# GemsLab/H2GCN

Measured on AMD Instinct MI355X. Metric: aggregated edges/sec (1+2-hop SpMM), higher is better.
Workload: dtype f32

## Files before the change

### h2gcn_amd/_capi.py

```python
from __future__ import annotations

import ctypes as C
import os
from pathlib import Path

ABI_VERSION = 4
MAX_HOPS = 8

OK = 0
ERR_INVALID_ARGUMENT = -1
ERR_HIP = -2
ERR_OUT_OF_MEMORY = -3
ERR_BAD_INDEX = -4
ERR_NO_TRANSPOSE = -5
ERR_INTERNAL = -6
ERR_EXCHANGE_TIMEOUT = -7

METRICS_MAX_SETS = 4
XCHG_BLOB_BYTES = 192
XCHG_COPY_ENGINE = 0
XCHG_COPY_KERNEL = 1

PLAN_BUILD_TRANSPOSE = 0x1
PLAN_SKIP_VALIDATION = 0x2
PLAN_HOST_TRANSPOSE = 0x4
PLAN_KEEP_PERMUTATION = 0x8

EXPORTED_SYMBOLS = (
    "h2gcn_abi_version",
    "h2gcn_last_error",
    "h2gcn_device_count",
    "h2gcn_plan_create",
    "h2gcn_plan_destroy",
    "h2gcn_plan_info",
    "h2gcn_plan_set_values",
    "h2gcn_spmm_hops_f32",
    "h2gcn_spmm_hops_T_f32",
    "h2gcn_plan_schedule",
    "h2gcn_plan_segment_classes",
    "h2gcn_spmm_workspace_bytes",
    "h2gcn_spmm_hops_opts_f32",
    "h2gcn_spmm_hops_T_opts_f32",
    "h2gcn_ring_scratch_bytes",
    "h2gcn_ring_count",
    "h2gcn_ring_fill",
    "h2gcn_ring_count_rows",
    "h2gcn_ring_fill_rows",
    "h2gcn_hop_normalize",
    "h2gcn_hop_normalize_rows",
    "h2gcn_dropout_dense_small_rows",
    "h2gcn_dropout_dense_workspace_bytes",
    "h2gcn_dropout_dense_f32",
    "h2gcn_dropout_dense_backward_f32",
    "h2gcn_masked_metrics_workspace_bytes",
    "h2gcn_masked_metrics_f32",
    "h2gcn_masked_ce_backward_f32",
    "h2gcn_adam_keras_f32",
    "h2gcn_adam_keras_l2_f32",
    "h2gcn_l2_penalty_workspace_bytes",
    "h2gcn_l2_penalty_f32",
    "h2gcn_xchg_create",
    "h2gcn_xchg_export",
    "h2gcn_xchg_connect",
    "h2gcn_xchg_allgather_begin",
    "h2gcn_xchg_allgather_post",
    "h2gcn_xchg_allgather_pull",
    "h2gcn_xchg_allgather_pull_rows",
    "h2gcn_xchg_allgather_end",
    "h2gcn_xchg_reduce_scatter_begin",
    "h2gcn_xchg_reduce_scatter_end",
    "h2gcn_xchg_reset_dependencies",
    "h2gcn_xchg_status",
    "h2gcn_xchg_destroy",
)


class PlanOpts(C.Structure):
    _fields_ = [
        ("struct_size", C.c_uint32),
        ("flags", C.c_uint32),
        ("long_row_threshold", C.c_int32),
        ("rows_per_wave", C.c_int32),
        ("variant", C.c_int32),
        ("slice_cols", C.c_int32),
        ("reserved", C.c_int32 * 2),
    ]


LAUNCH_RELU = 0x1
LAUNCH_ACCUMULATE = 0x2


class LaunchOpts(C.Structure):
    _fields_ = [
        ("struct_size", C.c_uint32),
        ("flags", C.c_uint32),
        ("workspace", C.c_void_p),
        ("workspace_bytes", C.c_size_t),
        ("bias", C.c_void_p),
    ]


class H2GCNError(RuntimeError):

    def __init__(self, status: int, message: str):
        super().__init__(f"libh2gcn_hip: {message} (status {status})")
        self.status = status


def library_path() -> Path:
    override = os.environ.get("H2GCN_HIP_LIBRARY")
    if override:
        return Path(override)
    return Path(__file__).resolve().parent / "csrc" / "libh2gcn_hip.so"


_LIB = None


def lib() -> C.CDLL:
    global _LIB
    if _LIB is not None:
        return _LIB
    path = library_path()
    if not path.exists():
        raise RuntimeError(
            f"{path} not found: build it with `python -c 'import __graft_entry__ as g; g.build()'` "
            "or `make -C h2gcn_amd/csrc`.  h2gcn_amd has no CPU fallback."
        )
    L = C.CDLL(str(path))
    L.h2gcn_abi_version.restype = C.c_int
    L.h2gcn_abi_version.argtypes = []
    L.h2gcn_last_error.restype = C.c_char_p
    L.h2gcn_last_error.argtypes = []
    L.h2gcn_device_count.restype = C.c_int
    L.h2gcn_device_count.argtypes = []
    L.h2gcn_plan_create.restype = C.c_int
    L.h2gcn_plan_create.argtypes = [
        C.c_int, C.c_int64, C.c_int64,
        C.POINTER(C.c_void_p), C.POINTER(C.c_void_p), C.POINTER(C.c_void_p),
        C.POINTER(PlanOpts), C.c_void_p, C.POINTER(C.c_void_p),
    ]
    L.h2gcn_plan_destroy.restype = None
    L.h2gcn_plan_destroy.argtypes = [C.c_void_p]
    L.h2gcn_plan_set_values.restype = C.c_int
    L.h2gcn_plan_set_values.argtypes = [C.c_void_p, C.c_int, C.c_void_p, C.c_void_p]
    L.h2gcn_plan_info.restype = C.c_int
    L.h2gcn_plan_info.argtypes = [
        C.c_void_p, C.c_int, C.POINTER(C.c_int64), C.POINTER(C.c_int64), C.POINTER(C.c_int64),
        C.POINTER(C.c_int64), C.POINTER(C.c_int32),
    ]
    L.h2gcn_spmm_hops_f32.restype = C.c_int
    L.h2gcn_spmm_hops_f32.argtypes = [
        C.c_void_p, C.c_uint32, C.c_void_p, C.c_int64, C.c_int32, C.c_void_p, C.c_int64, C.c_int64, C.c_void_p,
    ]
    L.h2gcn_spmm_hops_T_f32.restype = C.c_int
    L.h2gcn_spmm_hops_T_f32.argtypes = [
        C.c_void_p, C.c_uint32, C.c_void_p, C.c_int64, C.c_int64, C.c_int32, C.c_void_p, C.c_int64, C.c_void_p,
    ]
    L.h2gcn_plan_schedule.restype = C.c_int
    L.h2gcn_plan_schedule.argtypes = [C.c_void_p, C.c_uint32, C.c_int, C.c_int64, C.c_int32] + [C.POINTER(C.c_int32)] * 4
    if hasattr(L, "h2gcn_plan_segment_classes"):
        L.h2gcn_plan_segment_classes.restype = C.c_int
        L.h2gcn_plan_segment_classes.argtypes = [C.c_void_p, C.c_uint32, C.c_int, C.c_int64, C.c_int32] + [C.POINTER(C.c_int64)] * 3
    L.h2gcn_spmm_workspace_bytes.restype = C.c_size_t
    L.h2gcn_spmm_workspace_bytes.argtypes = [C.c_void_p, C.c_uint32, C.c_int, C.c_void_p, C.c_int64, C.c_int64, C.c_int32]
    L.h2gcn_spmm_hops_opts_f32.restype = C.c_int
    L.h2gcn_spmm_hops_opts_f32.argtypes = [
        C.c_void_p, C.c_uint32, C.c_void_p, C.c_int64, C.c_int32, C.c_void_p, C.c_int64, C.c_int64,
        C.POINTER(LaunchOpts), C.c_void_p,
    ]
    L.h2gcn_spmm_hops_T_opts_f32.restype = C.c_int
    L.h2gcn_spmm_hops_T_opts_f32.argtypes = [
        C.c_void_p, C.c_uint32, C.c_void_p, C.c_int64, C.c_int64, C.c_int32, C.c_void_p, C.c_int64,
        C.POINTER(LaunchOpts), C.c_void_p,
    ]
    L.h2gcn_ring_scratch_bytes.restype = C.c_size_t
    L.h2gcn_ring_scratch_bytes.argtypes = [C.c_int64]
    ring_common = [C.c_int64, C.c_void_p, C.c_void_p, C.c_void_p, C.c_void_p,
                   C.c_int, C.POINTER(C.c_void_p), C.POINTER(C.c_void_p), C.c_int,
                   C.c_int, C.POINTER(C.c_void_p), C.POINTER(C.c_void_p), C.c_int]
    L.h2gcn_ring_count.restype = C.c_int
    L.h2gcn_ring_count.argtypes = ring_common + [C.c_void_p, C.POINTER(C.c_int64), C.c_void_p, C.c_size_t, C.c_void_p]
    L.h2gcn_ring_fill.restype = C.c_int
    L.h2gcn_ring_fill.argtypes = ring_common + [C.c_void_p, C.c_void_p, C.c_void_p, C.c_size_t, C.c_void_p]
    ring_rows = [C.c_int64, C.c_int64, C.c_int64] + ring_common[1:]
    L.h2gcn_ring_count_rows.restype = C.c_int
    L.h2gcn_ring_count_rows.argtypes = ring_rows + [C.c_void_p, C.POINTER(C.c_int64), C.c_void_p, C.c_size_t, C.c_void_p]
    L.h2gcn_ring_fill_rows.restype = C.c_int
    L.h2gcn_ring_fill_rows.argtypes = ring_rows + [C.c_void_p, C.c_void_p, C.c_void_p, C.c_size_t, C.c_void_p]
    L.h2gcn_hop_normalize_rows.restype = C.c_int
    L.h2gcn_hop_normalize_rows.argtypes = [C.c_int64, C.c_void_p, C.c_void_p, C.c_int, C.c_void_p, C.c_int64, C.c_void_p, C.c_void_p, C.c_void_p]
    L.h2gcn_hop_normalize.restype = C.c_int
    L.h2gcn_hop_normalize.argtypes = [C.c_int64, C.c_void_p, C.c_void_p, C.c_int, C.c_void_p, C.c_int64, C.c_void_p, C.c_void_p]
    if hasattr(L, "h2gcn_dropout_dense_small_rows"):
        L.h2gcn_dropout_dense_small_rows.restype = C.c_int64
        L.h2gcn_dropout_dense_small_rows.argtypes = [C.c_int64]
    L.h2gcn_dropout_dense_workspace_bytes.restype = C.c_size_t
    L.h2gcn_dropout_dense_workspace_bytes.argtypes = [C.c_int64, C.c_int32, C.c_int32]
    L.h2gcn_dropout_dense_f32.restype = C.c_int
    L.h2gcn_dropout_dense_f32.argtypes = [C.c_void_p, C.c_int64, C.c_int64, C.c_int32, C.c_void_p, C.c_int32, C.c_void_p, C.c_float,
                                          C.c_uint64, C.c_void_p, C.c_void_p, C.c_int64, C.c_void_p, C.c_size_t, C.c_void_p]
    L.h2gcn_dropout_dense_backward_f32.restype = C.c_int
    L.h2gcn_dropout_dense_backward_f32.argtypes = [C.c_void_p, C.c_int64, C.c_int64, C.c_int32, C.c_void_p, C.c_int32, C.c_void_p, C.c_int64,
                                                   C.c_float, C.c_uint64, C.c_void_p, C.c_void_p, C.c_int64, C.c_void_p, C.c_void_p,
                                                   C.c_size_t, C.c_void_p]
    L.h2gcn_masked_metrics_workspace_bytes.restype = C.c_size_t
    L.h2gcn_masked_metrics_workspace_bytes.argtypes = [C.c_int64]
    L.h2gcn_masked_metrics_f32.restype = C.c_int
    L.h2gcn_masked_metrics_f32.argtypes = [C.c_void_p, C.c_int64, C.c_int64, C.c_int32, C.c_int32, C.POINTER(C.c_void_p), C.POINTER(C.c_int64),
                                           C.POINTER(C.c_void_p), C.c_void_p, C.c_void_p, C.c_void_p, C.c_size_t, C.c_void_p]
    L.h2gcn_masked_ce_backward_f32.restype = C.c_int
    L.h2gcn_masked_ce_backward_f32.argtypes = [C.c_void_p, C.c_int64, C.c_int64, C.c_int32, C.c_void_p, C.c_int64, C.c_void_p, C.c_void_p,
                                               C.c_void_p, C.c_int64, C.c_void_p]
    L.h2gcn_adam_keras_f32.restype = C.c_int
    L.h2gcn_adam_keras_f32.argtypes = [C.c_int32, C.POINTER(C.c_void_p), C.POINTER(C.c_void_p), C.POINTER(C.c_void_p), C.POINTER(C.c_void_p),
                                       C.POINTER(C.c_int64), C.c_float, C.c_float, C.c_float, C.c_float, C.c_void_p, C.c_int64, C.c_void_p]
    if hasattr(L, "h2gcn_adam_keras_l2_f32"):
        L.h2gcn_adam_keras_l2_f32.restype = C.c_int
        L.h2gcn_adam_keras_l2_f32.argtypes = [C.c_int32, C.POINTER(C.c_void_p), C.POINTER(C.c_void_p), C.POINTER(C.c_void_p), C.POINTER(C.c_void_p),
                                              C.POINTER(C.c_int64), C.POINTER(C.c_float), C.c_float, C.c_float, C.c_float, C.c_float, C.c_void_p,
                                              C.c_int64, C.c_void_p]
        L.h2gcn_l2_penalty_workspace_bytes.restype = C.c_size_t
        L.h2gcn_l2_penalty_workspace_bytes.argtypes = []
        L.h2gcn_l2_penalty_f32.restype = C.c_int
        L.h2gcn_l2_penalty_f32.argtypes = [C.c_int32, C.POINTER(C.c_void_p), C.POINTER(C.c_int64), C.POINTER(C.c_float), C.c_void_p, C.c_void_p,
                                           C.c_size_t, C.c_void_p]
    L.h2gcn_xchg_create.restype = C.c_int
    L.h2gcn_xchg_create.argtypes = [C.c_int, C.c_int, C.c_int, C.c_size_t, C.c_int, C.c_int, C.POINTER(C.c_void_p)]
    L.h2gcn_xchg_export.restype = C.c_int
    L.h2gcn_xchg_export.argtypes = [C.c_void_p, C.c_void_p]
    L.h2gcn_xchg_connect.restype = C.c_int
    L.h2gcn_xchg_connect.argtypes = [C.c_void_p, C.c_void_p]
    L.h2gcn_xchg_allgather_begin.restype = C.c_int
    L.h2gcn_xchg_allgather_begin.argtypes = [
        C.c_void_p, C.c_int, C.c_void_p, C.c_int64, C.c_int64, C.c_int64, C.c_int32, C.c_void_p, C.c_void_p,
    ]
    L.h2gcn_xchg_allgather_post.restype = C.c_int
    L.h2gcn_xchg_allgather_post.argtypes = L.h2gcn_xchg_allgather_begin.argtypes
    L.h2gcn_xchg_allgather_pull.restype = C.c_int
    L.h2gcn_xchg_allgather_pull.argtypes = [C.c_void_p, C.c_int, C.c_int64, C.c_int32, C.c_void_p]
    if hasattr(L, "h2gcn_xchg_allgather_pull_rows"):
        L.h2gcn_xchg_allgather_pull_rows.restype = C.c_int
        L.h2gcn_xchg_allgather_pull_rows.argtypes = [C.c_void_p, C.c_int, C.c_int64, C.c_int32, C.c_void_p, C.POINTER(C.c_void_p), C.POINTER(C.c_int64)]
    L.h2gcn_xchg_allgather_end.restype = C.c_int
    L.h2gcn_xchg_allgather_end.argtypes = [C.c_void_p, C.c_int, C.c_void_p]
    L.h2gcn_xchg_reduce_scatter_begin.restype = C.c_int
    L.h2gcn_xchg_reduce_scatter_begin.argtypes = [C.c_void_p, C.c_int, C.c_void_p, C.c_int64, C.c_int32, C.c_void_p, C.c_void_p]
    L.h2gcn_xchg_reduce_scatter_end.restype = C.c_int
    L.h2gcn_xchg_reduce_scatter_end.argtypes = [C.c_void_p, C.c_int, C.c_void_p]
    L.h2gcn_xchg_reset_dependencies.restype = C.c_int
    L.h2gcn_xchg_reset_dependencies.argtypes = [C.c_void_p]
    L.h2gcn_xchg_status.restype = C.c_int
    L.h2gcn_xchg_status.argtypes = [C.c_void_p]
    L.h2gcn_xchg_destroy.restype = None
    L.h2gcn_xchg_destroy.argtypes = [C.c_void_p]
    got = L.h2gcn_abi_version()
    if got != ABI_VERSION and not (os.environ.get("H2GCN_HIP_LIBRARY") and got == 3):
        raise RuntimeError(f"{path}: ABI version {got}, this front end expects {ABI_VERSION}")
    _LIB = L
    return L


def has(symbol: str) -> bool:
    return hasattr(lib(), symbol)


def check(status: int) -> None:
    if status < 0:
        msg = lib().h2gcn_last_error()
        raise H2GCNError(status, msg.decode("utf-8", "replace") if msg else "unknown error")
```

### h2gcn_amd/csrc/h2gcn_capi.hip

```cpp
#include <hip/hip_runtime.h>

#include <algorithm>
#include <cstdarg>
#include <cstdlib>
#include <cstdio>
#include <cstring>
#include <deque>
#include <map>
#include <mutex>
#include <memory>
#include <new>
#include <string>
#include <vector>

#include "h2gcn_hip.h"
#include "spmm_kernels.hip.h"

#include "capi_internal.h"

namespace h2gcn {

thread_local std::string g_last_error;

int fail(h2gcn_status st, const char* fmt, ...) {
    char buf[512];
    va_list ap;
    va_start(ap, fmt);
    vsnprintf(buf, sizeof(buf), fmt, ap);
    va_end(ap);
    g_last_error = buf;
    return (int)st;
}

}

namespace {

using h2gcn::fail;
using h2gcn::g_last_error;

struct DeviceBuf {
    void* p = nullptr;
    ~DeviceBuf() {
        if (p) (void)hipFree(p);
    }
    DeviceBuf() = default;
    DeviceBuf(DeviceBuf&& o) noexcept : p(o.p) { o.p = nullptr; }
    DeviceBuf(const DeviceBuf&) = delete;
    DeviceBuf& operator=(const DeviceBuf&) = delete;
};

struct HopOperand {
    const int64_t* rowptr = nullptr;
    const int32_t* colidx = nullptr;
    const float* vals = nullptr;
    int64_t nnz = 0;
    std::vector<int64_t> long_rows;
    std::vector<uint8_t> len8;
    int64_t n_short = 0, nnz_short = 0;
    int64_t nnz_long = 0;
    const uint32_t* perm = nullptr;
};

struct LongList {
    DeviceBuf dev;
    int n = 0;
    LongList() = default;
    LongList(LongList&&) noexcept = default;
};

struct ClassLists {
    DeviceBuf short_dev, med_dev;
    int64_t n_short = 0, nnz_short = 0, n_med = 0;
    bool built = false;
    ClassLists() = default;
    ClassLists(ClassLists&&) noexcept = default;
};

}

struct h2gcn_plan {
    int n_hops = 0;
    int64_t n_rows = 0, n_cols = 0;
    int long_threshold = 256;
    int rows_per_wave = 4;
    int variant = 0;
    int slice_cols = 0;
    bool has_transpose = false;
    int device = 0;
    std::vector<HopOperand> fwd;
    std::vector<HopOperand> adj;
    std::deque<DeviceBuf> owned;
    mutable std::mutex mu;
    mutable std::map<uint64_t, LongList> long_cache;
    mutable std::map<uint64_t, ClassLists> class_cache;
    int short_max = -1;
    double short_min_frac = 0.05;
};

namespace h2gcn {
__global__ void check_colidx_kernel(const int32_t* __restrict__ colidx, int64_t nnz, int64_t n_cols, int* flag) {
    int bad = 0;
    for (int64_t i = (int64_t)blockIdx.x * blockDim.x + threadIdx.x; i < nnz; i += (int64_t)gridDim.x * blockDim.x) {
        const int32_t c = colidx[i];
        bad |= (c < 0) | ((int64_t)c >= n_cols);
    }
    if (bad) atomicOr(flag, 1);
}

void launch_in_tile_short(bool sum, const LaunchParams& p, int slice, bool off32, bool fb4, dim3 grid, hipStream_t stream);
int transpose_csr_device(int64_t n_rows, int64_t n_cols, int64_t nnz, const int64_t* rowptr, const int32_t* colidx,
                         const float* vals, int64_t** t_rowptr_out, int32_t** t_colidx_out, float** t_vals_out,
                         uint32_t** perm_out_keep, hipStream_t stream, std::string* err);
void permute_values(const uint32_t* perm, const float* vals, int64_t nnz, float* t_vals, hipStream_t stream);
}

namespace {

using h2gcn::HopCsr;
using h2gcn::LaunchParams;

int transpose_csr_host(int64_t n_rows, int64_t n_cols, const std::vector<int64_t>& rowptr,
                       const std::vector<int32_t>& colidx, const std::vector<float>& vals,
                       std::vector<int64_t>& t_rowptr, std::vector<int32_t>& t_colidx, std::vector<float>& t_vals) {
    const int64_t nnz = rowptr[n_rows];
    t_rowptr.assign(n_cols + 1, 0);
    t_colidx.resize(nnz);
    t_vals.resize(nnz);
    for (int64_t i = 0; i < nnz; ++i) t_rowptr[colidx[i] + 1]++;
    for (int64_t c = 0; c < n_cols; ++c) t_rowptr[c + 1] += t_rowptr[c];
    std::vector<int64_t> cursor(t_rowptr.begin(), t_rowptr.end() - 1);
    for (int64_t r = 0; r < n_rows; ++r) {
        for (int64_t i = rowptr[r]; i < rowptr[r + 1]; ++i) {
            const int64_t dst = cursor[colidx[i]]++;
            t_colidx[dst] = (int32_t)r;
            t_vals[dst] = vals[i];
        }
    }
    return 0;
}

void collect_long_rows(const std::vector<int64_t>& rowptr, int64_t n_rows, int threshold, std::vector<int64_t>& out) {
    out.clear();
    for (int64_t r = 0; r < n_rows; ++r)
        if (rowptr[r + 1] - rowptr[r] >= threshold) out.push_back(r);
}

void collect_segment_lengths(const std::vector<int64_t>& rowptr, int64_t n_rows, int short_max, int long_threshold, HopOperand& op) {
    op.len8.resize((size_t)n_rows);
    op.n_short = op.nnz_short = op.nnz_long = 0;
    for (int64_t r = 0; r < n_rows; ++r) {
        const int64_t len = rowptr[r + 1] - rowptr[r];
        op.len8[(size_t)r] = (uint8_t)(len > 255 ? 255 : len);
        if (len <= short_max) {
            ++op.n_short;
            op.nnz_short += len;
        } else if (len >= long_threshold) {
            op.nnz_long += len;
        }
    }
}

thread_local bool t_stream_capturing = false;

struct CaptureScope {
    explicit CaptureScope(hipStream_t stream) {
        hipStreamCaptureStatus cs = hipStreamCaptureStatusNone;
        t_stream_capturing = hipStreamIsCapturing(stream, &cs) == hipSuccess && cs != hipStreamCaptureStatusNone;
        if (!t_stream_capturing) (void)hipGetLastError();
    }
    ~CaptureScope() { t_stream_capturing = false; }
};

int refuse_build_while_capturing(const char* what) {
    return fail(H2GCN_ERR_INVALID_ARGUMENT, "the stream is being captured and this is the first launch of this hop selection: its %s "
                "has to be built first (device allocation + upload).  Run the same launch once outside the capture (a warm-up step)", what);
}

int get_class_lists(const h2gcn_plan* plan, bool adjoint, int k, uint32_t mask, bool build, const ClassLists** out) {
    *out = nullptr;
    const std::vector<HopOperand>& ops = adjoint ? plan->adj : plan->fwd;
    const int64_t n_rows = adjoint ? plan->n_cols : plan->n_rows;
    if (plan->short_max < 0 || n_rows > 0x7fffffffLL) return H2GCN_OK;
    const uint64_t key = adjoint ? ((uint64_t)mask | (1ull << 32)) : ((uint64_t)k | (1ull << 40));
    const int sm = plan->short_max;
    std::lock_guard<std::mutex> lock(plan->mu);
    auto it = plan->class_cache.find(key);
    std::vector<const uint8_t*> sel;
    std::vector<uint8_t> any_long;
    auto prepare_adjoint = [&]() {
        any_long.assign((size_t)n_rows, 0);
        for (int h = 0; h < plan->n_hops; ++h)
            if (mask & (1u << h)) {
                sel.push_back(ops[h].len8.data());
                for (int64_t r : ops[h].long_rows) any_long[(size_t)r] = 1;
            }
    };
    if (it == plan->class_cache.end()) {
        ClassLists fresh;
        if (!adjoint) {
            fresh.n_short = ops[k].n_short;
            fresh.nnz_short = ops[k].nnz_short;
            fresh.n_med = n_rows - ops[k].n_short - (int64_t)ops[k].long_rows.size();
        } else {
            prepare_adjoint();
            for (int64_t r = 0; r < n_rows; ++r) {
                bool all = true;
                int64_t z = 0;
                for (const uint8_t* l : sel) { all = all && l[r] <= sm; z += l[r]; }
                if (all) { ++fresh.n_short; fresh.nnz_short += z; }
                else if (!any_long[(size_t)r]) ++fresh.n_med;
            }
        }
        it = plan->class_cache.emplace(key, std::move(fresh)).first;
    }
    ClassLists& cl = it->second;
    if (build && !cl.built) {
        if (t_stream_capturing) return refuse_build_while_capturing("per-class row lists");
        std::vector<int32_t> h_short, h_med;
        h_short.reserve((size_t)cl.n_short);
        h_med.reserve((size_t)cl.n_med);
        if (!adjoint) {
            const std::vector<uint8_t>& len = ops[k].len8;
            const std::vector<int64_t>& longs = ops[k].long_rows;
            size_t li = 0;
            for (int64_t r = 0; r < n_rows; ++r) {
                while (li < longs.size() && longs[li] < r) ++li;
                const bool is_long = li < longs.size() && longs[li] == r;
                if (len[(size_t)r] <= sm) h_short.push_back((int32_t)r);
                else if (!is_long) h_med.push_back((int32_t)r);
            }
        } else {
            if (sel.empty()) prepare_adjoint();
            for (int64_t r = 0; r < n_rows; ++r) {
                bool all = true;
                for (const uint8_t* l : sel) all = all && l[r] <= sm;
                if (all) h_short.push_back((int32_t)r);
                else if (!any_long[(size_t)r]) h_med.push_back((int32_t)r);
            }
        }
        DeviceBuf d_short, d_med;
        if (!h_short.empty()) {
            H2GCN_HIP_TRY(hipMalloc(&d_short.p, h_short.size() * sizeof(int32_t)));
            H2GCN_HIP_TRY(hipMemcpy(d_short.p, h_short.data(), h_short.size() * sizeof(int32_t), hipMemcpyHostToDevice));
        }
        if (!h_med.empty()) {
            H2GCN_HIP_TRY(hipMalloc(&d_med.p, h_med.size() * sizeof(int32_t)));
            H2GCN_HIP_TRY(hipMemcpy(d_med.p, h_med.data(), h_med.size() * sizeof(int32_t), hipMemcpyHostToDevice));
        }
        cl.short_dev.p = d_short.p;
        d_short.p = nullptr;
        cl.med_dev.p = d_med.p;
        d_med.p = nullptr;
        cl.built = true;
    }
    *out = &cl;
    return H2GCN_OK;
}

int check_rowptr(const std::vector<int64_t>& rowptr, int64_t n_rows, int hop) {
    if (rowptr[0] != 0) return fail(H2GCN_ERR_BAD_INDEX, "hop %d: rowptr[0] = %lld, expected 0", hop, (long long)rowptr[0]);
    for (int64_t r = 0; r < n_rows; ++r)
        if (rowptr[r + 1] < rowptr[r])
            return fail(H2GCN_ERR_BAD_INDEX, "hop %d: rowptr decreases at row %lld", hop, (long long)r);
    return H2GCN_OK;
}

int get_long_list(const h2gcn_plan* plan, bool adjoint, uint32_t mask, const int64_t** dev_out, int* n_out) {
    const uint64_t key = (uint64_t)mask | ((uint64_t)(adjoint ? 1 : 0) << 32);
    std::lock_guard<std::mutex> lock(plan->mu);
    auto it = plan->long_cache.find(key);
    if (it == plan->long_cache.end()) {
        const std::vector<HopOperand>& ops = adjoint ? plan->adj : plan->fwd;
        std::vector<int64_t> host;
        int s = 0;
        if (!adjoint) {
            for (int k = 0; k < plan->n_hops; ++k) {
                if (!(mask & (1u << k))) continue;
                for (int64_t r : ops[k].long_rows) host.push_back((r << 4) | s);
                ++s;
            }
        } else {
            for (int k = 0; k < plan->n_hops; ++k) {
                if (!(mask & (1u << k))) continue;
                host.insert(host.end(), ops[k].long_rows.begin(), ops[k].long_rows.end());
            }
            std::sort(host.begin(), host.end());
            host.erase(std::unique(host.begin(), host.end()), host.end());
        }
        LongList fresh;
        fresh.n = (int)host.size();
        if (fresh.n > 0 && t_stream_capturing) return refuse_build_while_capturing("long-segment list");
        if (fresh.n > 0) {
            H2GCN_HIP_TRY(hipMalloc(&fresh.dev.p, host.size() * sizeof(int64_t)));
            H2GCN_HIP_TRY(hipMemcpy(fresh.dev.p, host.data(), host.size() * sizeof(int64_t), hipMemcpyHostToDevice));
        }
        it = plan->long_cache.emplace(key, std::move(fresh)).first;
    }
    *dev_out = (const int64_t*)it->second.dev.p;
    *n_out = it->second.n;
    return H2GCN_OK;
}

constexpr int64_t kWavesToFill = 12288;

bool aligned16(const void* p) { return (reinterpret_cast<uintptr_t>(p) & 15u) == 0; }

int pick_slice_cols(int d, int64_t n_src_rows, int forced, double avg_segment_nnz, bool rows_line_aligned = false) {
    if (forced > 0) return forced;
    if (d < 64) return 64;
    static const int widths[] = {256, 128, 64};
    for (int w : widths) {
        if (d % w != 0) continue;
        const double slice_bytes = (double)n_src_rows * w * 4.0;
        if (w > 64 && avg_segment_nnz >= 16.0 && slice_bytes > 768.0 * 1024 * 1024 && d % (w / 2) == 0) continue;
        return w;
    }
    if (rows_line_aligned && d % 4 == 0 && avg_segment_nnz >= 16.0 && (double)n_src_rows * d * 4.0 >= 512.0 * 1024 * 1024) {
        return 64;
    }
    if (d > 256) {
        const bool beyond = avg_segment_nnz >= 16.0 && (double)n_src_rows * 256 * 4.0 > 768.0 * 1024 * 1024;
        return beyond ? 128 : 256;
    }
    int w = 64;
    while (w < d) w *= 2;
    return w;
}

struct LaunchShape {
    bool adjoint;
    int n_sel;
    int64_t nnz_sel;
    int64_t n_out, n_src;
    double avg;
    int64_t ld_src;
    int d;
    bool src_line_aligned;
    const int32_t* short_list[H2GCN_MAX_HOPS];
    int64_t short_count[H2GCN_MAX_HOPS];
    const int32_t* med_list[H2GCN_MAX_HOPS];
    int64_t med_count[H2GCN_MAX_HOPS];
    int n_short_lists;
    double short_frac;
    double short_nnz_frac;
};

LaunchShape shape_of(const h2gcn_plan* plan, uint32_t mask, bool adjoint);
int fill_short(const h2gcn_plan* plan, uint32_t mask, bool adjoint, LaunchShape& sh, bool build_lists = false);

int scratch_slice_cols(const h2gcn_plan* plan, const LaunchShape& sh) {
    if (plan->variant == 4) return 0;
    const int d = sh.d;
    if (sh.n_out == 0 || sh.n_src == 0 || sh.n_sel == 0) return 0;
    if (d <= 64) return 0;
    const double src_bytes = (double)sh.n_src * d * 4.0 * (sh.adjoint ? sh.n_sel : 1);
    if (src_bytes < 512.0 * 1024 * 1024) return 0;
    if ((double)sh.nnz_sel < 32.0 * (double)sh.n_src) return 0;
    if (!sh.adjoint && (sh.ld_src * 4) % 1024 == 0 && d % 64 == 0 && d >= 128) {
        const int w = pick_slice_cols(d, sh.n_src, plan->slice_cols, sh.avg);
        return (w == 64 || w == 128) && d % w == 0 && w < d ? w : 0;
    }
    if ((!sh.src_line_aligned || d % 4 != 0) && d > (sh.adjoint ? 256 : 128) && sh.avg >= 16.0 && (plan->slice_cols == 0 || plan->slice_cols == 64)) {
        return 64;
    }
    return 0;
}

size_t scratch_bytes(const LaunchShape& sh, int rs) {
    if (rs <= 0) return 0;
    const size_t n_slices = (size_t)((sh.d + rs - 1) / rs);
    return (size_t)sh.n_src * n_slices * (size_t)rs * 4 * (size_t)(sh.adjoint ? sh.n_sel : 1);
}

struct Schedule {
    bool pipe, scalar128, exact, shortrow, lists, fb4;
    int slice;
};

Schedule decide(int variant, bool exact_ok, int d, int rows_per_wave, int n_sel, int forced_slice, int64_t n_src_rows,
                double avg_segment_nnz, bool rows_line_aligned, bool gen, double short_frac, double short_nnz_frac, double short_min_frac,
                int64_t n_out_rows) {
    Schedule sc;
    if (variant == 4) variant = 0;
    sc.pipe = (variant == 2 || (variant == 0 && avg_segment_nnz < 16.0)) && rows_per_wave * n_sel <= 32;
    sc.scalar128 = exact_ok && variant == 1 && d == 128 && forced_slice == 0;
    sc.slice = (exact_ok && !sc.scalar128) ? pick_slice_cols(d, n_src_rows, forced_slice, avg_segment_nnz, rows_line_aligned) : 0;
    sc.exact = sc.slice > 0 || sc.scalar128;
    const bool grouped_ok = sc.exact && !sc.scalar128 && !gen && (sc.slice == 64 || sc.slice == 128);
    sc.shortrow = grouped_ok && (variant == 5 || (variant == 0 && avg_segment_nnz < 16.0 && n_out_rows >= 4 * kWavesToFill));
    sc.lists = grouped_ok && !sc.shortrow && short_frac > 0.0 && (variant == 6 || (variant == 0 && short_frac >= short_min_frac));
    sc.pipe = sc.pipe && sc.exact && !sc.shortrow && !sc.lists && !gen;
    const bool beyond = (double)n_src_rows * d * 4.0 >= 512.0 * 1024 * 1024;
    sc.fb4 = beyond && (sc.shortrow || (sc.lists && short_nnz_frac > 0.5));
    return sc;
}

template <bool SUM>
int launch(LaunchParams& p, const h2gcn_plan* plan, uint32_t mask, LaunchShape& sh, bool off32, int forced_slice, hipStream_t stream) {
    using namespace h2gcn;
    static const bool force_off64 = getenv("H2GCN_FORCE_OFF64") != nullptr;
    if (force_off64) off32 = false;
    const int variant = plan->variant;
    const bool exact_ok = p.d >= 4;
    const bool gen = p.d % 4 != 0 || p.bias != nullptr || p.relu != 0 || p.accumulate != 0;
    const Schedule sc = decide(variant, exact_ok, p.d, p.rows_per_wave, p.n_sel, forced_slice, sh.n_src, sh.avg,
                               sh.src_line_aligned, gen, sh.short_frac, sh.short_nnz_frac, plan->short_min_frac, sh.n_out);
    const bool short_fb4 = sc.fb4;
    const bool pipe = sc.pipe, scalar128 = sc.scalar128, exact = sc.exact, shortrow = sc.shortrow, lists = sc.lists;
    const int slice = sc.slice;
    p.slice_cols = exact ? (slice > 0 ? slice : 128) : p.d;
    p.n_slices = exact ? (p.d + p.slice_cols - 1) / p.slice_cols : 1;
    if (p.src_slice_stride == 0) p.src_slice_stride = p.slice_cols;
    p.short_max = -1;
    p.short_groups = p.med_groups = 0;
    if (lists) {
        int st = fill_short(plan, mask, SUM, sh, true);
        if (st != H2GCN_OK) return st;
        int64_t n_listed = 0, n_med = 0, longest = 0;
        for (int s = 0; s < sh.n_short_lists; ++s) {
            n_listed += sh.short_count[s];
            n_med += sh.med_count[s];
            longest = std::max(longest, sh.short_count[s]);
        }
        static const int env_mpw = getenv("H2GCN_MED_PER_WAVE") ? atoi(getenv("H2GCN_MED_PER_WAVE")) : 0;
        static const int env_spw = getenv("H2GCN_SHORT_PER_WAVE") ? atoi(getenv("H2GCN_SHORT_PER_WAVE")) : 0;
        static const int env_major = getenv("H2GCN_SHORT_HOP_MAJOR") ? atoi(getenv("H2GCN_SHORT_HOP_MAJOR")) : -1;
        const int mpw_max = SUM ? std::max(1, std::min(4, kWave / p.n_sel)) : 8;
        p.med_per_wave = (int)std::max<int64_t>(1, std::min<int64_t>(n_med / kWavesToFill, mpw_max));
        if (env_mpw >= 1 && env_mpw * p.n_sel <= kWave) p.med_per_wave = env_mpw;
        p.short_per_wave = 4;
        while (p.short_per_wave < 64 && n_listed / (2 * p.short_per_wave) >= kWavesToFill) p.short_per_wave *= 2;
        if (env_spw >= 4 && env_spw <= 64 && env_spw % 4 == 0) p.short_per_wave = env_spw;
        p.short_hop_major = env_major >= 0 ? env_major : 0;
        int64_t sblocks = 0, mblocks = 0;
        const int64_t s_per_block = (int64_t)kWavesPerBlock * p.short_per_wave;
        for (int s = 0; s < sh.n_short_lists; ++s) {
            p.short_list[s] = sh.short_list[s];
            p.short_count[s] = sh.short_count[s];
            sblocks += (sh.short_count[s] + s_per_block - 1) / s_per_block;
            p.short_end[s] = sblocks;
            p.med_list[s] = sh.med_list[s];
            p.med_count[s] = sh.med_count[s];
            const int64_t per_block = (int64_t)kWavesPerBlock * p.med_per_wave;
            mblocks += (sh.med_count[s] + per_block - 1) / per_block;
            p.med_end[s] = mblocks;
        }
        if (!SUM && !p.short_hop_major) sblocks = (longest + s_per_block - 1) / s_per_block * sh.n_short_lists;
        p.short_groups = (sblocks + kNumXcd - 1) / kNumXcd;
        p.med_groups = (mblocks + kNumXcd - 1) / kNumXcd;
        p.short_max = plan->short_max;
        p.blocks_per_slice = (int64_t)p.n_long + (p.short_groups + p.med_groups) * kNumXcd;
    } else {
        p.blocks_per_slice = (int64_t)p.n_long + p.tiles_per_xcd * kNumXcd;
    }
    const int64_t n_blocks = p.blocks_per_slice * p.n_slices;
    if (n_blocks <= 0) return H2GCN_OK;
    if (n_blocks > 0x7fffffffLL) return fail(H2GCN_ERR_INVALID_ARGUMENT, "grid too large (%lld blocks)", (long long)n_blocks);
    const dim3 grid((unsigned)n_blocks), block(kBlock);
#define H2GCN_LAUNCH_LISTS(VEC, LPR)                                                                                              \
    do {                                                                                                                          \
        if (off32 && short_fb4)                                                                                                   \
            hipLaunchKernelGGL((spmm_hops_kernel<VEC, LPR, true, SUM, true, false, false, false, 4, true>), grid, block, 0, stream, p);   \
        else if (off32)                                                                                                           \
            hipLaunchKernelGGL((spmm_hops_kernel<VEC, LPR, true, SUM, true, false, false, false, 8, true>), grid, block, 0, stream, p);   \
        else if (short_fb4)                                                                                                       \
            hipLaunchKernelGGL((spmm_hops_kernel<VEC, LPR, true, SUM, false, false, false, false, 4, true>), grid, block, 0, stream, p);  \
        else                                                                                                                      \
            hipLaunchKernelGGL((spmm_hops_kernel<VEC, LPR, true, SUM, false, false, false, false, 8, true>), grid, block, 0, stream, p);  \
    } while (0)
#define H2GCN_LAUNCH(VEC, LPR, EXACT)                                                                             \
    do {                                                                                                          \
        if (gen && off32)                                                                                         \
            hipLaunchKernelGGL((spmm_hops_kernel<VEC, LPR, EXACT, SUM, true, false, false, true>), grid, block, 0, stream, p);  \
        else if (gen)                                                                                             \
            hipLaunchKernelGGL((spmm_hops_kernel<VEC, LPR, EXACT, SUM, false, false, false, true>), grid, block, 0, stream, p); \
        else if (off32 && pipe && EXACT)                                                                               \
            hipLaunchKernelGGL((spmm_hops_kernel<VEC, LPR, EXACT, SUM, true, true>), grid, block, 0, stream, p);   \
        else if (off32)                                                                                           \
            hipLaunchKernelGGL((spmm_hops_kernel<VEC, LPR, EXACT, SUM, true, false>), grid, block, 0, stream, p);  \
        else if (pipe && EXACT)                                                                                   \
            hipLaunchKernelGGL((spmm_hops_kernel<VEC, LPR, EXACT, SUM, false, true>), grid, block, 0, stream, p);  \
        else                                                                                                      \
            hipLaunchKernelGGL((spmm_hops_kernel<VEC, LPR, EXACT, SUM, false, false>), grid, block, 0, stream, p); \
    } while (0)
    if (scalar128) {
        H2GCN_LAUNCH(2, 64, true);
    } else if (slice == 256) {
        H2GCN_LAUNCH(4, 64, true);
    } else if (slice == 128 && lists) {
        H2GCN_LAUNCH_LISTS(4, 32);
    } else if (slice == 64 && lists) {
        H2GCN_LAUNCH_LISTS(4, 16);
    } else if ((slice == 128 || slice == 64) && shortrow) {
        launch_in_tile_short(SUM, p, slice, off32, short_fb4, grid, stream);
    } else if (slice == 128) {
        H2GCN_LAUNCH(4, 32, true);
    } else if (slice == 64) {
        H2GCN_LAUNCH(4, 16, true);
    } else {
        H2GCN_LAUNCH(1, 64, false);
    }
#undef H2GCN_LAUNCH
#undef H2GCN_LAUNCH_LISTS
    H2GCN_HIP_TRY(hipGetLastError());
    return H2GCN_OK;
}

void use_scratch(LaunchParams& p, const LaunchShape& sh, int rs, int64_t ld_src_hop, void* workspace, hipStream_t stream,
                 bool* off32) {
    const int n_hop = sh.adjoint ? sh.n_sel : 1;
    const int n_slices = (sh.d + rs - 1) / rs;
    const bool vec4 = sh.d % 4 == 0;
    const int64_t total = sh.n_src * (int64_t)n_slices * n_hop * (rs / (vec4 ? 4 : 1));
    const unsigned blocks = (unsigned)std::min<int64_t>((total + 255) / 256, 256 * 64);
    if (vec4)
        hipLaunchKernelGGL(h2gcn::repack_slice_major_kernel<true>, dim3(blocks), dim3(256), 0, stream, p.src, sh.ld_src,
                           ld_src_hop, n_hop, sh.n_src, sh.d, n_slices, rs, (float*)workspace);
    else
        hipLaunchKernelGGL(h2gcn::repack_slice_major_kernel<false>, dim3(blocks), dim3(256), 0, stream, p.src, sh.ld_src,
                           ld_src_hop, n_hop, sh.n_src, sh.d, n_slices, rs, (float*)workspace);
    p.src = (const float*)workspace;
    p.ld_src = rs;
    p.d_src = (sh.d + 3) & ~3;
    p.src_slice_stride = sh.n_src * (int64_t)rs * n_hop;
    for (int s = 0; s < p.n_sel; ++s) p.src_hop_off[s] = sh.adjoint ? (int64_t)s * sh.n_src * rs : 0;
    *off32 = (double)sh.n_src * (double)n_slices * rs * n_hop * 4.0 < 4294967296.0;
}

int check_device(const h2gcn_plan* plan) {
    int cur = -1;
    H2GCN_HIP_TRY(hipGetDevice(&cur));
    if (cur != plan->device)
        return fail(H2GCN_ERR_INVALID_ARGUMENT, "plan lives on device %d but the current HIP device is %d", plan->device, cur);
    return H2GCN_OK;
}

int resolve_mask(const h2gcn_plan* plan, uint32_t hop_mask, uint32_t* out) {
    const uint32_t all = plan->n_hops >= 32 ? 0xffffffffu : ((1u << plan->n_hops) - 1u);
    if (hop_mask == 0) hop_mask = all;
    if (hop_mask & ~all) return fail(H2GCN_ERR_INVALID_ARGUMENT, "hop_mask 0x%x selects hops beyond the plan's %d", hop_mask, plan->n_hops);
    *out = hop_mask;
    return H2GCN_OK;
}

}

extern "C" {

int h2gcn_abi_version(void) { return H2GCN_ABI_VERSION; }

const char* h2gcn_last_error(void) { return g_last_error.c_str(); }

int h2gcn_device_count(void) {
    int n = 0;
    hipError_t e = hipGetDeviceCount(&n);
    if (e != hipSuccess) return fail(H2GCN_ERR_HIP, "hipGetDeviceCount failed: %s", hipGetErrorString(e));
    return n;
}

int h2gcn_plan_create(int n_hops, int64_t n_rows, int64_t n_cols, const int64_t* const* rowptr_dev,
                      const int32_t* const* colidx_dev, const float* const* vals_dev,
                      const h2gcn_plan_opts* opts, void* stream_v, h2gcn_plan_t** out_plan) {
    try {
        if (!out_plan) return fail(H2GCN_ERR_INVALID_ARGUMENT, "out_plan is NULL");
        *out_plan = nullptr;
        if (n_hops < 1 || n_hops > H2GCN_MAX_HOPS)
            return fail(H2GCN_ERR_INVALID_ARGUMENT, "n_hops = %d, supported 1..%d", n_hops, H2GCN_MAX_HOPS);
        if (n_rows < 0 || n_cols < 0 || n_cols > 0x7fffffffLL)
            return fail(H2GCN_ERR_INVALID_ARGUMENT, "bad shape %lld x %lld (column ids are int32)", (long long)n_rows, (long long)n_cols);
        if (n_rows >= (1LL << 58)) return fail(H2GCN_ERR_INVALID_ARGUMENT, "n_rows too large");
        if (!rowptr_dev || !colidx_dev || !vals_dev) return fail(H2GCN_ERR_INVALID_ARGUMENT, "NULL operand table");
        h2gcn_plan_opts o;
        memset(&o, 0, sizeof(o));
        if (opts) {
            if (opts->struct_size < 8 || opts->struct_size > sizeof(o))
                return fail(H2GCN_ERR_INVALID_ARGUMENT, "opts->struct_size = %u", opts->struct_size);
            memcpy(&o, opts, opts->struct_size);
        }
        if (o.slice_cols != 0 && o.slice_cols != 64 && o.slice_cols != 128 && o.slice_cols != 256)
            return fail(H2GCN_ERR_INVALID_ARGUMENT, "slice_cols = %d, supported 0 (auto), 64, 128, 256", o.slice_cols);
        if (o.long_row_threshold < 0 || o.rows_per_wave < 0 || o.rows_per_wave > h2gcn::kMaxRowsPerWave)
            return fail(H2GCN_ERR_INVALID_ARGUMENT, "bad tunable (long_row_threshold %d, rows_per_wave %d, max %d)",
                        o.long_row_threshold, o.rows_per_wave, h2gcn::kMaxRowsPerWave);
        hipStream_t stream = (hipStream_t)stream_v;

        std::unique_ptr<h2gcn_plan> plan(new h2gcn_plan());
        plan->n_hops = n_hops;
        plan->n_rows = n_rows;
        plan->n_cols = n_cols;
        if (o.long_row_threshold > 0) plan->long_threshold = o.long_row_threshold;
        if (o.rows_per_wave > 0) plan->rows_per_wave = o.rows_per_wave;
        else if (const char* e = getenv("H2GCN_ROWS_PER_WAVE")) plan->rows_per_wave = std::max(1, std::min(atoi(e), h2gcn::kMaxRowsPerWave));
        else {
            plan->rows_per_wave = (int)std::max<int64_t>(1, std::min<int64_t>(n_rows / kWavesToFill, 4));
        }
        while ((plan->rows_per_wave + 1) * n_hops > h2gcn::kWave && plan->rows_per_wave > 1) plan->rows_per_wave--;
        plan->variant = o.variant;
        if (o.variant == 0) if (const char* e = getenv("H2GCN_VARIANT")) plan->variant = atoi(e);
        plan->slice_cols = o.slice_cols;
        if (o.slice_cols == 0) if (const char* e = getenv("H2GCN_SLICE_COLS")) plan->slice_cols = atoi(e);
        plan->short_max = std::min(h2gcn::kShortMax, plan->long_threshold - 1);
        if (const char* e = getenv("H2GCN_SHORT_MIN_FRAC")) plan->short_min_frac = atof(e);
        H2GCN_HIP_TRY(hipGetDevice(&plan->device));
        plan->fwd.resize(n_hops);

        DeviceBuf flag;
        H2GCN_HIP_TRY(hipMalloc(&flag.p, sizeof(int)));
        H2GCN_HIP_TRY(hipMemsetAsync(flag.p, 0, sizeof(int), stream));

        std::vector<std::vector<int64_t>> h_rowptr(n_hops);
        for (int k = 0; k < n_hops; ++k) {
            if (!rowptr_dev[k]) return fail(H2GCN_ERR_INVALID_ARGUMENT, "hop %d: rowptr is NULL", k);
            h_rowptr[k].resize(n_rows + 1);
            H2GCN_HIP_TRY(hipMemcpyAsync(h_rowptr[k].data(), rowptr_dev[k], (n_rows + 1) * sizeof(int64_t), hipMemcpyDeviceToHost, stream));
        }
        H2GCN_HIP_TRY(hipStreamSynchronize(stream));
        for (int k = 0; k < n_hops; ++k) {
            int st = check_rowptr(h_rowptr[k], n_rows, k);
            if (st != H2GCN_OK) return st;
            HopOperand& op = plan->fwd[k];
            op.rowptr = rowptr_dev[k];
            op.colidx = colidx_dev[k];
            op.vals = vals_dev[k];
            op.nnz = h_rowptr[k][n_rows];
            if (op.nnz > 0 && (!op.colidx || !op.vals)) return fail(H2GCN_ERR_INVALID_ARGUMENT, "hop %d: colidx/vals is NULL", k);
            collect_long_rows(h_rowptr[k], n_rows, plan->long_threshold, op.long_rows);
            collect_segment_lengths(h_rowptr[k], n_rows, plan->short_max, plan->long_threshold, op);
            if (!(o.flags & H2GCN_PLAN_SKIP_VALIDATION) && op.nnz > 0) {
                const int64_t want = (op.nnz + 255) / 256;
                const unsigned blocks = (unsigned)std::min<int64_t>(want, 4096);
                hipLaunchKernelGGL(h2gcn::check_colidx_kernel, dim3(blocks), dim3(256), 0, stream, op.colidx, op.nnz, n_cols, (int*)flag.p);
                H2GCN_HIP_TRY(hipGetLastError());
            }
        }
        int h_flag = 0;
        H2GCN_HIP_TRY(hipMemcpyAsync(&h_flag, flag.p, sizeof(int), hipMemcpyDeviceToHost, stream));
        H2GCN_HIP_TRY(hipStreamSynchronize(stream));
        if (h_flag) return fail(H2GCN_ERR_BAD_INDEX, "a column index lies outside [0, %lld)", (long long)n_cols);

        if (o.flags & H2GCN_PLAN_BUILD_TRANSPOSE) {
            if (n_rows > 0x7fffffffLL) return fail(H2GCN_ERR_INVALID_ARGUMENT, "transpose needs n_rows < 2^31");
            plan->adj.resize(n_hops);
            for (int k = 0; k < n_hops; ++k) {
                const int64_t nnz = plan->fwd[k].nnz;
                int64_t* t_rp = nullptr;
                int32_t* t_ci = nullptr;
                float* t_va = nullptr;
                uint32_t* t_perm = nullptr;
                const bool keep_perm = (o.flags & H2GCN_PLAN_KEEP_PERMUTATION) != 0;
                if (keep_perm && (o.flags & H2GCN_PLAN_HOST_TRANSPOSE))
                    return fail(H2GCN_ERR_INVALID_ARGUMENT, "H2GCN_PLAN_KEEP_PERMUTATION needs the device transposition");
                std::vector<int64_t> t_rowptr(n_cols + 1);
                std::string terr;
                int st = (o.flags & H2GCN_PLAN_HOST_TRANSPOSE)
                             ? -1
                             : h2gcn::transpose_csr_device(n_rows, n_cols, nnz, rowptr_dev[k], colidx_dev[k], vals_dev[k],
                                                           &t_rp, &t_ci, &t_va, keep_perm ? &t_perm : nullptr, stream, &terr);
                if (st != 0 && keep_perm && st != -3)
                    return fail(H2GCN_ERR_INVALID_ARGUMENT, "H2GCN_PLAN_KEEP_PERMUTATION: %s", terr.c_str());
                if (st == 0) {
                    plan->owned.emplace_back(); plan->owned.back().p = t_rp;
                    plan->owned.emplace_back(); plan->owned.back().p = t_ci;
                    plan->owned.emplace_back(); plan->owned.back().p = t_va;
                    plan->owned.emplace_back(); plan->owned.back().p = t_perm;
                    H2GCN_HIP_TRY(hipMemcpy(t_rowptr.data(), t_rp, (n_cols + 1) * sizeof(int64_t), hipMemcpyDeviceToHost));
                } else if (st == -3) {
                    return fail(H2GCN_ERR_OUT_OF_MEMORY, "transposition of hop %d: %s", k, terr.c_str());
                } else {
                    std::vector<int32_t> h_col(nnz);
                    std::vector<float> h_val(nnz);
                    if (nnz > 0) {
                        H2GCN_HIP_TRY(hipMemcpy(h_col.data(), colidx_dev[k], nnz * sizeof(int32_t), hipMemcpyDeviceToHost));
                        H2GCN_HIP_TRY(hipMemcpy(h_val.data(), vals_dev[k], nnz * sizeof(float), hipMemcpyDeviceToHost));
                    }
                    std::vector<int32_t> t_col;
                    std::vector<float> t_val;
                    transpose_csr_host(n_rows, n_cols, h_rowptr[k], h_col, h_val, t_rowptr, t_col, t_val);
                    plan->owned.emplace_back();
                    DeviceBuf& d_rp = plan->owned.back();
                    H2GCN_HIP_TRY(hipMalloc(&d_rp.p, (n_cols + 1) * sizeof(int64_t)));
                    H2GCN_HIP_TRY(hipMemcpy(d_rp.p, t_rowptr.data(), (n_cols + 1) * sizeof(int64_t), hipMemcpyHostToDevice));
                    plan->owned.emplace_back();
                    DeviceBuf& d_ci = plan->owned.back();
                    plan->owned.emplace_back();
                    DeviceBuf& d_va = plan->owned.back();
                    if (nnz > 0) {
                        H2GCN_HIP_TRY(hipMalloc(&d_ci.p, nnz * sizeof(int32_t)));
                        H2GCN_HIP_TRY(hipMemcpy(d_ci.p, t_col.data(), nnz * sizeof(int32_t), hipMemcpyHostToDevice));
                        H2GCN_HIP_TRY(hipMalloc(&d_va.p, nnz * sizeof(float)));
                        H2GCN_HIP_TRY(hipMemcpy(d_va.p, t_val.data(), nnz * sizeof(float), hipMemcpyHostToDevice));
                    }
                    t_rp = (int64_t*)d_rp.p;
                    t_ci = (int32_t*)d_ci.p;
                    t_va = (float*)d_va.p;
                }
                HopOperand& op = plan->adj[k];
                op.rowptr = t_rp;
                op.colidx = t_ci;
                op.vals = t_va;
                op.nnz = nnz;
                op.perm = t_perm;
                collect_long_rows(t_rowptr, n_cols, plan->long_threshold, op.long_rows);
                collect_segment_lengths(t_rowptr, n_cols, plan->short_max, plan->long_threshold, op);
            }
            plan->has_transpose = true;
        }
        {
            const uint32_t all = n_hops >= 32 ? 0xffffffffu : ((1u << n_hops) - 1u);
            const int64_t* unused_p = nullptr;
            int unused_n = 0;
            int st = get_long_list(plan.get(), false, all, &unused_p, &unused_n);
            if (st == H2GCN_OK && plan->has_transpose) st = get_long_list(plan.get(), true, all, &unused_p, &unused_n);
            if (st != H2GCN_OK) return st;
            auto mixed = [&](const LaunchShape& sh_) {
                return plan->variant == 6 || (plan->variant == 0 && sh_.short_frac >= plan->short_min_frac &&
                                              (sh_.avg >= 16.0 || sh_.n_out < 4 * kWavesToFill));
            };
            LaunchShape sh_f = shape_of(plan.get(), all, false);
            if ((st = fill_short(plan.get(), all, false, sh_f)) != H2GCN_OK) return st;
            if (mixed(sh_f) && (st = fill_short(plan.get(), all, false, sh_f, true)) != H2GCN_OK) return st;
            if (plan->has_transpose) {
                LaunchShape sh_a = shape_of(plan.get(), all, true);
                if ((st = fill_short(plan.get(), all, true, sh_a)) != H2GCN_OK) return st;
                if (mixed(sh_a) && (st = fill_short(plan.get(), all, true, sh_a, true)) != H2GCN_OK) return st;
            }
        }
        *out_plan = plan.release();
        return H2GCN_OK;
    } catch (const std::bad_alloc&) {
        return fail(H2GCN_ERR_OUT_OF_MEMORY, "host allocation failed in plan_create");
    } catch (...) {
        return fail(H2GCN_ERR_INTERNAL, "unexpected exception in plan_create");
    }
}

void h2gcn_plan_destroy(h2gcn_plan_t* plan) { delete plan; }

int h2gcn_plan_set_values(h2gcn_plan_t* plan, int hop, const float* vals_dev, void* stream_v) {
    if (!plan) return fail(H2GCN_ERR_INVALID_ARGUMENT, "plan is NULL");
    if (hop < 0 || hop >= plan->n_hops) return fail(H2GCN_ERR_INVALID_ARGUMENT, "hop %d outside 0..%d", hop, plan->n_hops - 1);
    HopOperand& f = plan->fwd[hop];
    if (f.nnz > 0 && !vals_dev) return fail(H2GCN_ERR_INVALID_ARGUMENT, "vals is NULL");
    int st = check_device(plan);
    if (st != H2GCN_OK) return st;
    if (plan->has_transpose) {
        HopOperand& a = plan->adj[hop];
        if (a.nnz > 0 && !a.perm)
            return fail(H2GCN_ERR_INVALID_ARGUMENT, "plan has transposed operands but was created without H2GCN_PLAN_KEEP_PERMUTATION");
        h2gcn::permute_values(a.perm, vals_dev, a.nnz, const_cast<float*>(a.vals), (hipStream_t)stream_v);
        H2GCN_HIP_TRY(hipGetLastError());
    }
    f.vals = vals_dev;
    return H2GCN_OK;
}

int h2gcn_plan_info(const h2gcn_plan_t* plan, int hop, int64_t* n_rows, int64_t* n_cols, int64_t* nnz,
                    int64_t* n_long_segments, int32_t* has_transpose) {
    if (!plan) return fail(H2GCN_ERR_INVALID_ARGUMENT, "plan is NULL");
    if (hop < 0 || hop >= plan->n_hops) return fail(H2GCN_ERR_INVALID_ARGUMENT, "hop %d outside 0..%d", hop, plan->n_hops - 1);
    if (n_rows) *n_rows = plan->n_rows;
    if (n_cols) *n_cols = plan->n_cols;
    if (nnz) *nnz = plan->fwd[hop].nnz;
    if (n_long_segments) *n_long_segments = (int64_t)plan->fwd[hop].long_rows.size();
    if (has_transpose) *has_transpose = plan->has_transpose ? 1 : 0;
    return H2GCN_OK;
}

namespace {
bool line_aligned(const float* src, int64_t ld_src, int64_t ld_src_hop, int n_sel, bool adjoint) {
    return (reinterpret_cast<uintptr_t>(src) & 127u) == 0 && (ld_src * 4) % 128 == 0 && (!adjoint || n_sel <= 1 || (ld_src_hop * 4) % 128 == 0);
}

LaunchShape shape_of(const h2gcn_plan* plan, uint32_t mask, bool adjoint) {
    LaunchShape sh;
    memset(&sh, 0, sizeof(sh));
    sh.adjoint = adjoint;
    const std::vector<HopOperand>& ops = adjoint ? plan->adj : plan->fwd;
    for (int k = 0; k < plan->n_hops; ++k)
        if (mask & (1u << k)) { sh.nnz_sel += ops[k].nnz; ++sh.n_sel; }
    sh.n_out = adjoint ? plan->n_cols : plan->n_rows;
    sh.n_src = adjoint ? plan->n_rows : plan->n_cols;
    sh.avg = (sh.n_out > 0 && sh.n_sel > 0) ? (double)sh.nnz_sel / ((double)sh.n_out * sh.n_sel) : 0.0;
    return sh;
}

int fill_short(const h2gcn_plan* plan, uint32_t mask, bool adjoint, LaunchShape& sh, bool build_lists) {
    sh.n_short_lists = 0;
    sh.short_frac = sh.short_nnz_frac = 0.0;
    if (plan->short_max < 0 || sh.n_out <= 0 || sh.n_sel <= 0) return H2GCN_OK;
    int64_t n = 0, nnz = 0;
    const ClassLists* cl = nullptr;
    if (!adjoint) {
        int s = 0;
        for (int k = 0; k < plan->n_hops; ++k) {
            if (!(mask & (1u << k))) continue;
            int st = get_class_lists(plan, false, k, 0, build_lists, &cl);
            if (st != H2GCN_OK) return st;
            if (!cl) return H2GCN_OK;
            sh.short_list[s] = (const int32_t*)cl->short_dev.p;
            sh.short_count[s] = cl->n_short;
            sh.med_list[s] = (const int32_t*)cl->med_dev.p;
            sh.med_count[s] = cl->n_med;
            n += cl->n_short;
            nnz += cl->nnz_short;
            ++s;
        }
        sh.n_short_lists = s;
        sh.short_frac = (double)n / ((double)sh.n_out * sh.n_sel);
    } else {
        if (sh.n_sel > h2gcn::kShortSumHops) return H2GCN_OK;
        int st = get_class_lists(plan, true, 0, mask, build_lists, &cl);
        if (st != H2GCN_OK) return st;
        if (!cl) return H2GCN_OK;
        sh.short_list[0] = (const int32_t*)cl->short_dev.p;
        sh.short_count[0] = cl->n_short;
        sh.med_list[0] = (const int32_t*)cl->med_dev.p;
        sh.med_count[0] = cl->n_med;
        n = cl->n_short;
        nnz = cl->nnz_short;
        sh.n_short_lists = 1;
        sh.short_frac = (double)n / (double)sh.n_out;
    }
    if (n == 0) sh.n_short_lists = 0;
    sh.short_nnz_frac = sh.nnz_sel > 0 ? (double)nnz / (double)sh.nnz_sel : (n > 0 ? 1.0 : 0.0);
    return H2GCN_OK;
}

}

int h2gcn_plan_schedule(const h2gcn_plan_t* plan, uint32_t hop_mask, int adjoint, int64_t ld_src, int32_t d,
                        int32_t* slice_cols, int32_t* n_slices, int32_t* segment_walk, int32_t* scratch_copy) {
    if (!plan) return fail(H2GCN_ERR_INVALID_ARGUMENT, "plan is NULL");
    uint32_t mask;
    int st = resolve_mask(plan, hop_mask, &mask);
    if (st != H2GCN_OK) return st;
    if (d < 1 || ld_src < d) return fail(H2GCN_ERR_INVALID_ARGUMENT, "bad width %d / stride %lld", d, (long long)ld_src);
    if (adjoint && !plan->has_transpose) return fail(H2GCN_ERR_NO_TRANSPOSE, "plan was created without H2GCN_PLAN_BUILD_TRANSPOSE");
    LaunchShape sh = shape_of(plan, mask, adjoint != 0);
    if ((st = fill_short(plan, mask, adjoint != 0, sh)) != H2GCN_OK) return st;
    sh.ld_src = ld_src;
    sh.d = d;
    sh.src_line_aligned = (ld_src * 4) % 128 == 0 && (!adjoint || sh.n_sel <= 1 || (d * 4) % 128 == 0);
    const int rs = scratch_slice_cols(plan, sh);
    const Schedule sc = decide(plan->variant, d >= 4, d, plan->rows_per_wave, sh.n_sel, rs > 0 ? rs : plan->slice_cols, sh.n_src, sh.avg,
                               rs > 0 || sh.src_line_aligned, d % 4 != 0, sh.short_frac, sh.short_nnz_frac, plan->short_min_frac, sh.n_out);
    const int w = sc.exact ? (sc.slice > 0 ? sc.slice : 128) : d;
    if (slice_cols) *slice_cols = w;
    if (n_slices) *n_slices = sc.exact ? (d + w - 1) / w : 1;
    if (segment_walk) *segment_walk = sc.pipe ? 1 : (sc.shortrow ? 2 : (sc.lists ? 3 : 0));
    if (scratch_copy) *scratch_copy = rs > 0 ? 1 : 0;
    return H2GCN_OK;
}

int h2gcn_plan_segment_classes(const h2gcn_plan_t* plan, uint32_t hop_mask, int adjoint, int64_t ld_src, int32_t d,
                               int64_t* segments, int64_t* nonzeros, int64_t* listed) {
    if (!plan) return fail(H2GCN_ERR_INVALID_ARGUMENT, "plan is NULL");
    uint32_t mask;
    int st = resolve_mask(plan, hop_mask, &mask);
    if (st != H2GCN_OK) return st;
    if (d < 1 || ld_src < d) return fail(H2GCN_ERR_INVALID_ARGUMENT, "bad width %d / stride %lld", d, (long long)ld_src);
    if (adjoint && !plan->has_transpose) return fail(H2GCN_ERR_NO_TRANSPOSE, "plan was created without H2GCN_PLAN_BUILD_TRANSPOSE");
    const std::vector<HopOperand>& ops = adjoint ? plan->adj : plan->fwd;
    const int64_t n_out = adjoint ? plan->n_cols : plan->n_rows;
    int s = 0;
    for (int k = 0; k < plan->n_hops; ++k) {
        if (!(mask & (1u << k))) continue;
        const HopOperand& op = ops[k];
        const int64_t n_long = (int64_t)op.long_rows.size();
        if (segments) {
            segments[3 * s + 0] = op.n_short;
            segments[3 * s + 1] = n_out - op.n_short - n_long;
            segments[3 * s + 2] = n_long;
        }
        if (nonzeros) {
            nonzeros[3 * s + 0] = op.nnz_short;
            nonzeros[3 * s + 1] = op.nnz - op.nnz_short - op.nnz_long;
            nonzeros[3 * s + 2] = op.nnz_long;
        }
        ++s;
    }
    if (listed) {
        LaunchShape sh = shape_of(plan, mask, adjoint != 0);
        if ((st = fill_short(plan, mask, adjoint != 0, sh)) != H2GCN_OK) return st;
        sh.ld_src = ld_src;
        sh.d = d;
        sh.src_line_aligned = (ld_src * 4) % 128 == 0 && (!adjoint || sh.n_sel <= 1 || (d * 4) % 128 == 0);
        const int rs = scratch_slice_cols(plan, sh);
        const Schedule sc = decide(plan->variant, d >= 4, d, plan->rows_per_wave, sh.n_sel, rs > 0 ? rs : plan->slice_cols, sh.n_src, sh.avg,
                                   rs > 0 || sh.src_line_aligned, d % 4 != 0, sh.short_frac, sh.short_nnz_frac, plan->short_min_frac, sh.n_out);
        *listed = 0;
        if (sc.lists)
            for (int q = 0; q < sh.n_short_lists; ++q) *listed += sh.short_count[q];
        if (sc.shortrow) *listed = -1;
    }
    return H2GCN_OK;
}

size_t h2gcn_spmm_workspace_bytes(const h2gcn_plan_t* plan, uint32_t hop_mask, int adjoint, const float* src_dev,
                                  int64_t ld_src, int64_t ld_src_hop, int32_t d) {
    if (!plan || d < 1 || ld_src < d) return 0;
    if (adjoint && !plan->has_transpose) return 0;
    uint32_t mask;
    if (resolve_mask(plan, hop_mask, &mask) != H2GCN_OK) return 0;
    LaunchShape sh = shape_of(plan, mask, adjoint != 0);
    sh.src_line_aligned = line_aligned(src_dev, ld_src, ld_src_hop, sh.n_sel, adjoint != 0);
    sh.ld_src = ld_src;
    sh.d = d;
    return scratch_bytes(sh, scratch_slice_cols(plan, sh));
}

int h2gcn_spmm_hops_f32(const h2gcn_plan_t* plan, uint32_t hop_mask, const float* X, int64_t ldx, int32_t d,
                        float* Y, int64_t ldy_row, int64_t ldy_hop, void* stream_v) {
    return h2gcn_spmm_hops_opts_f32(plan, hop_mask, X, ldx, d, Y, ldy_row, ldy_hop, nullptr, stream_v);
}

namespace {
int read_launch_opts(const h2gcn_launch_opts* lopts, h2gcn_launch_opts* lo) {
    memset(lo, 0, sizeof(*lo));
    if (lopts) {
        if (lopts->struct_size < 8 || lopts->struct_size > sizeof(*lo))
            return fail(H2GCN_ERR_INVALID_ARGUMENT, "launch opts struct_size = %u", lopts->struct_size);
        memcpy(lo, lopts, lopts->struct_size);
    }
    if (lo->flags & ~(uint32_t)(H2GCN_LAUNCH_RELU | H2GCN_LAUNCH_ACCUMULATE)) return fail(H2GCN_ERR_INVALID_ARGUMENT, "unknown launch flags 0x%x", lo->flags);
    return H2GCN_OK;
}
}

int h2gcn_spmm_hops_opts_f32(const h2gcn_plan_t* plan, uint32_t hop_mask, const float* X, int64_t ldx, int32_t d,
                             float* Y, int64_t ldy_row, int64_t ldy_hop, const h2gcn_launch_opts* lopts,
                             void* stream_v) {
    try {
        h2gcn_launch_opts lo;
        int st = read_launch_opts(lopts, &lo);
        if (st != H2GCN_OK) return st;
        if (lo.flags & ~H2GCN_LAUNCH_RELU) return fail(H2GCN_ERR_INVALID_ARGUMENT, "forward launch flags 0x%x: only H2GCN_LAUNCH_RELU applies", lo.flags);
        if (!plan) return fail(H2GCN_ERR_INVALID_ARGUMENT, "plan is NULL");
        uint32_t mask;
        st = resolve_mask(plan, hop_mask, &mask);
        if (st != H2GCN_OK) return st;
        if ((st = check_device(plan)) != H2GCN_OK) return st;
        if (d < 1) return fail(H2GCN_ERR_INVALID_ARGUMENT, "d = %d", d);
        if (plan->n_rows == 0) return H2GCN_OK;
        if (!Y) return fail(H2GCN_ERR_INVALID_ARGUMENT, "Y is NULL");
        if (!X && plan->n_cols > 0) return fail(H2GCN_ERR_INVALID_ARGUMENT, "X is NULL");
        if (ldx < d) return fail(H2GCN_ERR_INVALID_ARGUMENT, "ldx = %lld < d = %d", (long long)ldx, d);
        if (ldy_hop < 0 || ldy_row < 0) return fail(H2GCN_ERR_INVALID_ARGUMENT, "negative output stride");
        CaptureScope capture_scope((hipStream_t)stream_v);
        LaunchParams p;
        memset(&p, 0, sizeof(p));
        LaunchShape sh = shape_of(plan, mask, false);
        int s = 0;
        for (int k = 0; k < plan->n_hops; ++k) {
            if (!(mask & (1u << k))) continue;
            const HopOperand& op = plan->fwd[k];
            p.hop[s] = HopCsr{op.rowptr, op.colidx, op.vals};
            p.src_hop_off[s] = 0;
            p.dst_hop_off[s] = (int64_t)s * ldy_hop;
            ++s;
        }
        p.n_sel = s;
        if (s > 1 && ldy_hop < d) return fail(H2GCN_ERR_INVALID_ARGUMENT, "ldy_hop = %lld < d = %d: hop outputs would overlap", (long long)ldy_hop, d);
        p.d = d;
        p.d_src = d;
        p.n_rows = plan->n_rows;
        p.src = X;
        p.ld_src = ldx;
        p.dst = Y;
        p.ld_dst = ldy_row;
        p.bias = lo.bias_dev;
        p.relu = (lo.flags & H2GCN_LAUNCH_RELU) ? 1 : 0;
        st = get_long_list(plan, false, mask, &p.long_list, &p.n_long);
        if (st != H2GCN_OK) return st;
        p.long_threshold = plan->long_threshold;
        p.rows_per_wave = plan->rows_per_wave;
        const int64_t rows_per_tile = (int64_t)p.rows_per_wave * h2gcn::kWavesPerBlock;
        p.n_tiles = (p.n_rows + rows_per_tile - 1) / rows_per_tile;
        p.tiles_per_xcd = (p.n_tiles + h2gcn::kNumXcd - 1) / h2gcn::kNumXcd;
        bool off32 = ((double)(plan->n_cols > 0 ? plan->n_cols - 1 : 0) * (double)ldx + d) * 4.0 < 4294967296.0;
        int forced_slice = plan->slice_cols;
        sh.ld_src = ldx;
        sh.d = d;
        sh.src_line_aligned = line_aligned(X, ldx, 0, s, false);
        const int rs = (lo.workspace_dev && aligned16(lo.workspace_dev)) ? scratch_slice_cols(plan, sh) : 0;
        if (rs > 0 && lo.workspace_bytes >= scratch_bytes(sh, rs)) {
            use_scratch(p, sh, rs, 0, lo.workspace_dev, (hipStream_t)stream_v, &off32);
            H2GCN_HIP_TRY(hipGetLastError());
            forced_slice = rs;
        }
        if ((st = fill_short(plan, mask, false, sh)) != H2GCN_OK) return st;
        return launch<false>(p, plan, mask, sh, off32, forced_slice, (hipStream_t)stream_v);
    } catch (...) {
        return fail(H2GCN_ERR_INTERNAL, "unexpected exception in spmm_hops_opts_f32");
    }
}

int h2gcn_spmm_hops_T_f32(const h2gcn_plan_t* plan, uint32_t hop_mask, const float* dY, int64_t ldg_row,
                          int64_t ldg_hop, int32_t d, float* dX, int64_t ldx, void* stream_v) {
    return h2gcn_spmm_hops_T_opts_f32(plan, hop_mask, dY, ldg_row, ldg_hop, d, dX, ldx, nullptr, stream_v);
}

int h2gcn_spmm_hops_T_opts_f32(const h2gcn_plan_t* plan, uint32_t hop_mask, const float* dY, int64_t ldg_row,
                               int64_t ldg_hop, int32_t d, float* dX, int64_t ldx, const h2gcn_launch_opts* lopts,
                               void* stream_v) {
    try {
        h2gcn_launch_opts lo;
        int st = read_launch_opts(lopts, &lo);
        if (st != H2GCN_OK) return st;
        if (lo.bias_dev || (lo.flags & ~H2GCN_LAUNCH_ACCUMULATE))
            return fail(H2GCN_ERR_INVALID_ARGUMENT, "the adjoint launch has no bias / activation epilogue (only H2GCN_LAUNCH_ACCUMULATE is accepted)");
        if (!plan) return fail(H2GCN_ERR_INVALID_ARGUMENT, "plan is NULL");
        if (!plan->has_transpose)
            return fail(H2GCN_ERR_NO_TRANSPOSE, "plan was created without H2GCN_PLAN_BUILD_TRANSPOSE");
        uint32_t mask;
        st = resolve_mask(plan, hop_mask, &mask);
        if (st != H2GCN_OK) return st;
        if ((st = check_device(plan)) != H2GCN_OK) return st;
        if (d < 1) return fail(H2GCN_ERR_INVALID_ARGUMENT, "d = %d", d);
        if (plan->n_cols == 0) return H2GCN_OK;
        if (!dX) return fail(H2GCN_ERR_INVALID_ARGUMENT, "dX is NULL");
        if (!dY && plan->n_rows > 0) return fail(H2GCN_ERR_INVALID_ARGUMENT, "dY is NULL");
        if (ldx < d) return fail(H2GCN_ERR_INVALID_ARGUMENT, "ldx = %lld < d = %d", (long long)ldx, d);
        if (ldg_row < d || ldg_hop < 0) return fail(H2GCN_ERR_INVALID_ARGUMENT, "bad gradient strides");
        CaptureScope capture_scope((hipStream_t)stream_v);
        LaunchParams p;
        memset(&p, 0, sizeof(p));
        LaunchShape sh = shape_of(plan, mask, true);
        int s = 0;
        for (int k = 0; k < plan->n_hops; ++k) {
            if (!(mask & (1u << k))) continue;
            const HopOperand& op = plan->adj[k];
            p.hop[s] = HopCsr{op.rowptr, op.colidx, op.vals};
            p.src_hop_off[s] = (int64_t)s * ldg_hop;
            p.dst_hop_off[s] = 0;
            ++s;
        }
        p.n_sel = s;
        p.d = d;
        p.d_src = d;
        p.n_rows = plan->n_cols;
        p.src = dY;
        p.ld_src = ldg_row;
        p.dst = dX;
        p.ld_dst = ldx;
        p.accumulate = (lo.flags & H2GCN_LAUNCH_ACCUMULATE) ? 1 : 0;
        st = get_long_list(plan, true, mask, &p.long_list, &p.n_long);
        if (st != H2GCN_OK) return st;
        p.long_threshold = plan->long_threshold;
        p.rows_per_wave = plan->rows_per_wave;
        const int64_t rows_per_tile = (int64_t)p.rows_per_wave * h2gcn::kWavesPerBlock;
        p.n_tiles = (p.n_rows + rows_per_tile - 1) / rows_per_tile;
        p.tiles_per_xcd = (p.n_tiles + h2gcn::kNumXcd - 1) / h2gcn::kNumXcd;
        bool off32 = ((double)(plan->n_rows > 0 ? plan->n_rows - 1 : 0) * (double)ldg_row + (double)(s - 1) * (double)ldg_hop + d) * 4.0 < 4294967296.0;
        int forced_slice = plan->slice_cols;
        sh.ld_src = ldg_row;
        sh.d = d;
        sh.src_line_aligned = line_aligned(dY, ldg_row, ldg_hop, s, true);
        const int rs = (lo.workspace_dev && aligned16(lo.workspace_dev) && plan->n_rows > 0) ? scratch_slice_cols(plan, sh) : 0;
        if (rs > 0 && lo.workspace_bytes >= scratch_bytes(sh, rs)) {
            use_scratch(p, sh, rs, ldg_hop, lo.workspace_dev, (hipStream_t)stream_v, &off32);
            H2GCN_HIP_TRY(hipGetLastError());
            forced_slice = rs;
        }
        if ((st = fill_short(plan, mask, true, sh)) != H2GCN_OK) return st;
        return launch<true>(p, plan, mask, sh, off32, forced_slice, (hipStream_t)stream_v);
    } catch (...) {
        return fail(H2GCN_ERR_INTERNAL, "unexpected exception in spmm_hops_T_f32");
    }
}

}
```

### h2gcn_amd/csrc/spmm_kernels.hip.h

```cpp
#pragma once

#include <hip/hip_runtime.h>
#include <stdint.h>

#include <type_traits>

#include "h2gcn_hip.h"

namespace h2gcn {

constexpr int kWave = 64;
constexpr int kWavesPerBlock = 4;
constexpr int kBlock = kWave * kWavesPerBlock;
constexpr int kNumXcd = 8;
constexpr int kMaxRowsPerWave = 7;
#ifndef H2GCN_MIN_WAVES
#define H2GCN_MIN_WAVES 6
#endif
constexpr int kMinWavesPerSimd = H2GCN_MIN_WAVES;
#ifndef H2GCN_SHORT_MIN_WAVES
#define H2GCN_SHORT_MIN_WAVES 4
#endif
#ifndef H2GCN_SHORT_FB4_MIN_WAVES
#define H2GCN_SHORT_FB4_MIN_WAVES 7
#endif
#ifndef H2GCN_MAIN_MAXB
#define H2GCN_MAIN_MAXB 8
#endif
#ifndef H2GCN_WIDE_MAXB
#define H2GCN_WIDE_MAXB H2GCN_MAIN_MAXB
#endif
#ifndef H2GCN_WIDE_MIN_WAVES
#define H2GCN_WIDE_MIN_WAVES H2GCN_MIN_WAVES
#endif
constexpr int kShortMax = 16;
constexpr int kShortSumHops = 4;
#ifndef H2GCN_SHORT_PREFETCH
#define H2GCN_SHORT_PREFETCH 2
#endif
#ifndef H2GCN_OFF64_HEAVY_MIN_WAVES
#define H2GCN_OFF64_HEAVY_MIN_WAVES 5
#endif
constexpr int kMaxTileCols = 256;
constexpr int kTreeParts = 4;

template <int LPR>
struct Tree {
    static constexpr int G = kWave / LPR;
    static_assert(G == 1 || G == 2 || G == 4, "lane geometries: 64 / 128 / 256 columns per slice");
    static constexpr int NP = kTreeParts / G;
};

struct HopCsr {
    const int64_t* rowptr;
    const int32_t* colidx;
    const float* vals;
};

struct LaunchParams {
    HopCsr hop[H2GCN_MAX_HOPS];
    int64_t src_hop_off[H2GCN_MAX_HOPS];
    int64_t dst_hop_off[H2GCN_MAX_HOPS];
    int n_sel;
    int d;
    int d_src;
    int64_t n_rows;
    const float* src;
    int64_t ld_src;
    int64_t src_slice_stride;
    float* dst;
    int64_t ld_dst;
    const int64_t* long_list;
    int n_long;
    int long_threshold;
    int rows_per_wave;
    int64_t n_tiles;
    int64_t tiles_per_xcd;
    int n_slices;
    int slice_cols;
    int64_t blocks_per_slice;
    const float* bias;
    int relu;
    int accumulate;
    const int32_t* short_list[H2GCN_MAX_HOPS];
    int64_t short_count[H2GCN_MAX_HOPS];
    int64_t short_end[H2GCN_MAX_HOPS];
    int64_t short_groups;
    int short_max;
    int short_per_wave;
    int short_hop_major;
    const int32_t* med_list[H2GCN_MAX_HOPS];
    int64_t med_count[H2GCN_MAX_HOPS];
    int64_t med_end[H2GCN_MAX_HOPS];
    int64_t med_groups;
    int med_per_wave;
};

template <int VEC>
struct VecT;
template <>
struct VecT<1> {
    using type = float;
};
template <>
struct VecT<2> {
    typedef float type __attribute__((ext_vector_type(2), aligned(4)));
};
template <>
struct VecT<4> {
    typedef float type __attribute__((ext_vector_type(4), aligned(4)));
};

__device__ __forceinline__ int wave_uniform(int v) { return __builtin_amdgcn_readfirstlane(v); }

__device__ __forceinline__ int lane_gather(int v, int src_lane) {
    return __builtin_amdgcn_ds_bpermute(src_lane << 2, v);
}
__device__ __forceinline__ float lane_gather(float v, int src_lane) {
    return __int_as_float(__builtin_amdgcn_ds_bpermute(src_lane << 2, __float_as_int(v)));
}

__device__ __forceinline__ float fold_xor32(float v) {
    const unsigned u = __float_as_uint(v);
    auto r = __builtin_amdgcn_permlane32_swap(u, u, false, false);
    return __uint_as_float(r[0]) + __uint_as_float(r[1]);
}
__device__ __forceinline__ float fold_xor16(float v) {
    const unsigned u = __float_as_uint(v);
    auto r = __builtin_amdgcn_permlane16_swap(u, u, false, false);
    return __uint_as_float(r[0]) + __uint_as_float(r[1]);
}
__device__ __forceinline__ float fold_xor8(float v) {
    const int o = __builtin_amdgcn_update_dpp(0, __float_as_int(v), 0x128 , 0xf, 0xf, false);
    return v + __int_as_float(o);
}

__device__ __forceinline__ float fold_ror4(float v) {
    const int o = __builtin_amdgcn_update_dpp(0, __float_as_int(v), 0x124 , 0xf, 0xf, false);
    return v + __int_as_float(o);
}

template <int LPR>
__device__ __forceinline__ float fold_groups(float v) {
    if constexpr (LPR <= 8) v = fold_xor8(v);
    if constexpr (LPR <= 4) v = fold_ror4(v);
    if constexpr (LPR <= 16) v = fold_xor16(v);
    if constexpr (LPR <= 32) v = fold_xor32(v);
    return v;
}

template <int VEC, int LPR, int NP>
__device__ __forceinline__ void fold_tree(const float (&acc)[NP][VEC], float (&tot)[VEC]) {
    constexpr int G = kWave / LPR;
    static_assert(NP == Tree<LPR>::NP, "partials per lane");
#pragma unroll
    for (int i = 0; i < VEC; ++i) {
        if constexpr (G == 1) tot[i] = (acc[0][i] + acc[1][i]) + (acc[2][i] + acc[3][i]);
        else if constexpr (G == 2) tot[i] = fold_xor32(acc[0][i]) + fold_xor32(acc[1][i]);
        else tot[i] = fold_groups<LPR>(acc[0][i]);
    }
}

template <int VEC, int NP>
__device__ __forceinline__ void zero_acc(float (&acc)[NP][VEC]) {
#pragma unroll
    for (int k = 0; k < NP; ++k)
#pragma unroll
        for (int i = 0; i < VEC; ++i) acc[k][i] = 0.f;
}

template <int VEC>
__device__ __forceinline__ typename VecT<VEC>::type load_vec(const float* p) {
#ifdef H2GCN_NT_GATHER
    return __builtin_nontemporal_load(reinterpret_cast<const typename VecT<VEC>::type*>(p));
#else
    return *reinterpret_cast<const typename VecT<VEC>::type*>(p);
#endif
}

template <int VEC>
__device__ __forceinline__ void fma_vec(float (&acc)[VEC], float w, typename VecT<VEC>::type x) {
    if constexpr (VEC == 1) {
        acc[0] = fmaf(w, x, acc[0]);
    } else {
#pragma unroll
        for (int i = 0; i < VEC; ++i) acc[i] = fmaf(w, x[i], acc[i]);
    }
}

template <bool OFF32>
struct GatherAddr {
    const char* base;
    typename std::conditional<OFF32, uint32_t, int64_t>::type lane_off;
    typename std::conditional<OFF32, uint32_t, int64_t>::type ld_bytes;
    __device__ __forceinline__ const float* row(int col) const {
        if constexpr (OFF32) {
            return reinterpret_cast<const float*>(base + (uint32_t)(lane_off + (uint32_t)col * ld_bytes));
        } else {
            return reinterpret_cast<const float*>(base + (lane_off + (int64_t)col * ld_bytes));
        }
    }
};

template <int VEC, int LPR, int U, bool PREDICATED, bool OFF32, int PHASE = 0, int NP>
__device__ __forceinline__ void gather_batch(int c, float v, int t, int g, const GatherAddr<OFF32>& addr, bool take,
                                             float (&acc)[NP][VEC]) {
    constexpr int G = kWave / LPR;
    typename VecT<VEC>::type x[U];
    float w[U];
#pragma unroll
    for (int u = 0; u < U; ++u) {
        int cj;
        if constexpr (G == 1) {
            cj = __builtin_amdgcn_readlane(c, t + u);
            w[u] = __int_as_float(__builtin_amdgcn_readlane(__float_as_int(v), t + u));
        } else {
            const int idx = ((t + u) * G + g) & (kWave - 1);
            cj = lane_gather(c, idx);
            w[u] = lane_gather(v, idx);
        }
        const float* p = addr.row(cj);
        if constexpr (PREDICATED) {
            if (take) {
                x[u] = load_vec<VEC>(p);
            } else {
                w[u] = 0.f;
                if constexpr (VEC == 1) x[u] = 0.f; else x[u] = (typename VecT<VEC>::type)(0.f);
            }
        } else {
            x[u] = load_vec<VEC>(p);
        }
    }
#pragma unroll
    for (int u = 0; u < U; ++u) fma_vec<VEC>(acc[(PHASE + u) % NP], w[u], x[u]);
}

__device__ __forceinline__ void load_chunk(const int32_t* __restrict__ colidx, const float* __restrict__ vals,
                                           int64_t base, int64_t seg_end, int lane, int& c, float& v) {
    c = 0;
    v = 0.f;
    if (base + lane < seg_end) {
        c = __builtin_nontemporal_load(colidx + base + lane);
        v = __builtin_nontemporal_load(vals + base + lane);
    }
}

template <int VEC, int LPR, bool MASKED, bool OFF32, int MAXB = H2GCN_MAIN_MAXB, int NP>
__device__ __forceinline__ void process_chunk(int c, float v, int n, int g, const GatherAddr<OFF32>& addr,
                                              bool lane_active, float (&acc)[NP][VEC]) {
    constexpr int G = kWave / LPR;
    const int full = n / G;
    int t = 0;
    if constexpr (MAXB >= 8)
        for (; t + 8 <= full; t += 8) gather_batch<VEC, LPR, 8, MASKED, OFF32>(c, v, t, g, addr, lane_active, acc);
    if constexpr (MAXB < 8)
        for (; t + 4 <= full; t += 4) gather_batch<VEC, LPR, 4, MASKED, OFF32>(c, v, t, g, addr, lane_active, acc);
    if (t + 4 <= full) {
        gather_batch<VEC, LPR, 4, MASKED, OFF32>(c, v, t, g, addr, lane_active, acc);
        t += 4;
    }
    const int rem = n - full * G;
    if (t + 2 <= full) {
        gather_batch<VEC, LPR, 2, MASKED, OFF32>(c, v, t, g, addr, lane_active, acc);
        t += 2;
        if (t + 1 <= full) {
            gather_batch<VEC, LPR, 1, MASKED, OFF32, 2 % NP>(c, v, t, g, addr, lane_active, acc);
            if constexpr (G > 1)
                if (rem > 0) gather_batch<VEC, LPR, 1, true, OFF32, 3 % NP>(c, v, full, g, addr, lane_active && g < rem, acc);
        } else {
            if constexpr (G > 1)
                if (rem > 0) gather_batch<VEC, LPR, 1, true, OFF32, 2 % NP>(c, v, full, g, addr, lane_active && g < rem, acc);
        }
    } else if (t + 1 <= full) {
        gather_batch<VEC, LPR, 1, MASKED, OFF32>(c, v, t, g, addr, lane_active, acc);
        if constexpr (G > 1)
            if (rem > 0) gather_batch<VEC, LPR, 1, true, OFF32, 1 % NP>(c, v, full, g, addr, lane_active && g < rem, acc);
    } else {
        if constexpr (G > 1)
            if (rem > 0) gather_batch<VEC, LPR, 1, true, OFF32>(c, v, full, g, addr, lane_active && g < rem, acc);
    }
}

template <int VEC, int LPR, bool MASKED, bool OFF32, int MAXB = H2GCN_MAIN_MAXB, int NP>
__device__ __forceinline__ void accumulate_segment(const int32_t* __restrict__ colidx,
                                                   const float* __restrict__ vals, int64_t seg_begin,
                                                   int64_t seg_end, int chunk0, int chunk_step,
                                                   const GatherAddr<OFF32>& addr, int lane, bool lane_active,
                                                   float (&acc)[NP][VEC]) {
    const int g = lane / LPR;
    for (int64_t base = seg_begin + (int64_t)chunk0 * kWave; base < seg_end; base += (int64_t)chunk_step * kWave) {
        const int64_t left = seg_end - base;
        const int n = left < kWave ? (int)left : kWave;
        int c;
        float v;
        load_chunk(colidx, vals, base, seg_end, lane, c, v);
        process_chunk<VEC, LPR, MASKED, OFF32, MAXB>(c, v, n, g, addr, lane_active, acc);
    }
}

template <int VEC, int LPR, bool OFF32, int MAXB = H2GCN_MAIN_MAXB, int NP>
__device__ __forceinline__ void accumulate_segment_prefetched(const int32_t* __restrict__ colidx,
                                                              const float* __restrict__ vals, int64_t seg_begin,
                                                              int64_t seg_end, int c, float v,
                                                              const GatherAddr<OFF32>& addr, int lane,
                                                              float (&acc)[NP][VEC]) {
    const int g = lane / LPR;
    for (int64_t base = seg_begin; base < seg_end; base += kWave) {
        const int64_t left = seg_end - base;
        const int n = left < kWave ? (int)left : kWave;
        int c_next = 0;
        float v_next = 0.f;
        if (left > kWave) load_chunk(colidx, vals, base + kWave, seg_end, lane, c_next, v_next);
        process_chunk<VEC, LPR, false, OFF32, MAXB>(c, v, n, g, addr, true, acc);
        c = c_next;
        v = v_next;
    }
}

template <int VEC, int LPR, bool OFF32>
__device__ __forceinline__ void accumulate_grouped(int c, float v, int n_mine, int n_max, int lane,
                                                   const GatherAddr<OFF32>& addr, float (&part)[kTreeParts][VEC]) {
    constexpr int U = kTreeParts;
    const int group_base = lane & ~(LPR - 1);
    for (int t = 0; t < n_max; t += U) {
        typename VecT<VEC>::type x[U];
        float w[U];
#pragma unroll
        for (int u = 0; u < U; ++u) {
            const int cj = lane_gather(c, group_base + t + u);
            w[u] = lane_gather(v, group_base + t + u);
            if (t + u < n_mine) {
                x[u] = load_vec<VEC>(addr.row(cj));
            } else {
                w[u] = 0.f;
                if constexpr (VEC == 1) x[u] = 0.f; else x[u] = (typename VecT<VEC>::type)(0.f);
            }
        }
#pragma unroll
        for (int u = 0; u < U; ++u)
            if (t + u < n_mine) fma_vec<VEC>(part[u], w[u], x[u]);
    }
}

template <int VEC>
__device__ __forceinline__ void combine_partials(const float (&part)[kTreeParts][VEC], float (&acc)[VEC]) {
#pragma unroll
    for (int i = 0; i < VEC; ++i) acc[i] = (part[0][i] + part[1][i]) + (part[2][i] + part[3][i]);
}

template <int VEC>
__device__ __forceinline__ void epilogue(float (&acc)[VEC], const float* __restrict__ bias, int relu, int col) {
    if (bias) {
#pragma unroll
        for (int i = 0; i < VEC; ++i) acc[i] += bias[col + i];
    }
    if (relu) {
#pragma unroll
        for (int i = 0; i < VEC; ++i) acc[i] = fmaxf(acc[i], 0.f);
    }
}

template <int VEC>
__device__ __forceinline__ void store_vec(float* p, const float (&acc)[VEC]) {
    if constexpr (VEC == 1) {
        __builtin_nontemporal_store(acc[0], p);
    } else {
        typename VecT<VEC>::type o;
#pragma unroll
        for (int i = 0; i < VEC; ++i) o[i] = acc[i];
#if defined(H2GCN_AB_NO_STORES)
        if (acc[0] == 1.2345678e30f)
            __builtin_nontemporal_store(o, reinterpret_cast<typename VecT<VEC>::type*>(p));
#elif defined(H2GCN_PLAIN_STORES)
        *reinterpret_cast<typename VecT<VEC>::type*>(p) = o;
#else
        __builtin_nontemporal_store(o, reinterpret_cast<typename VecT<VEC>::type*>(p));
#endif
    }
}

template <int VEC, bool GEN, typename P>
__device__ __forceinline__ void store_out(const P& p, float* row, int col0, int ecol, float (&tot)[VEC]) {
    if (col0 + VEC <= p.d) {
        if constexpr (GEN) {
            if (p.accumulate) {
                if constexpr (VEC == 1) {
                    tot[0] += row[col0];
                } else {
                    const typename VecT<VEC>::type old = *reinterpret_cast<const typename VecT<VEC>::type*>(row + col0);
#pragma unroll
                    for (int i = 0; i < VEC; ++i) tot[i] += old[i];
                }
            }
            epilogue<VEC>(tot, p.bias, p.relu, col0);
        }
        store_vec<VEC>(row + col0, tot);
        return;
    }
    if constexpr (GEN) {
        if (col0 < p.d) {
#pragma unroll
            for (int i = 0; i < VEC; ++i) {
                const int c = ecol + i;
                if (c >= col0 && c < p.d) {
                    float t = tot[i];
                    if (p.accumulate) t += row[c];
                    if (p.bias) t += p.bias[c];
                    if (p.relu) t = fmaxf(t, 0.f);
                    __builtin_nontemporal_store(t, row + c);
                }
            }
        }
    }
}

template <int VEC, int LPR, bool SUM, bool OFF32, bool EPI, int PD>
__device__ __forceinline__ void short_list_blocks(const LaunchParams& p, int64_t sblock, int lane, int wave, int64_t lane_off0,
                                                  int64_t src_col_begin, int lcol, int ecol,
                                                  uint64_t (&s_seg)[kWavesPerBlock][kShortSumHops][kWave],
                                                  int32_t (&s_row)[kWavesPerBlock][kWave]) {
    using off_t = typename std::conditional<OFF32, uint32_t, int64_t>::type;
    constexpr int G = kWave / LPR;
    constexpr uint64_t kBeginMask = (1ull << 58) - 1;
    const int li = lane % LPR, g = lane / LPR;
    const int n_sel = p.n_sel;
    int hop = 0;
    int64_t local = sblock;
    if constexpr (!SUM) {
        if (p.short_hop_major) {
            while (hop + 1 < n_sel && sblock >= p.short_end[hop]) ++hop;
            if (hop > 0) local -= p.short_end[hop - 1];
        } else {
            local = sblock / n_sel;
            hop = (int)(sblock - local * n_sel);
        }
    }
    const int spw = p.short_per_wave;
    const int64_t entry0 = (local * kWavesPerBlock + wave) * spw;
    const int64_t left = p.short_count[hop] - entry0;
    if (left <= 0) return;
    const int n_here = left < spw ? (int)left : spw;
    const int NS = SUM ? n_sel : 1;
    if (lane < n_here) {
        const int32_t row = __builtin_nontemporal_load(p.short_list[hop] + entry0 + lane);
        s_row[wave][lane] = row;
        for (int s = 0; s < NS; ++s) {
            const int64_t* rp = p.hop[SUM ? s : hop].rowptr + row;
            const int64_t b0 = rp[0], b1 = rp[1];
            s_seg[wave][s][lane] = (uint64_t)b0 | ((uint64_t)(b1 - b0) << 58);
        }
    }
    __builtin_amdgcn_fence(__ATOMIC_RELEASE, "wavefront");
    __builtin_amdgcn_wave_barrier();
    __builtin_amdgcn_fence(__ATOMIC_ACQUIRE, "wavefront");
    const int n_rounds = (n_here + G - 1) / G;
    const int n_steps = n_rounds * NS;

    int cq[PD], lq[PD];
    float vq[PD];
    int ft = 0, fs = 0;
    auto fetch = [&](int& c, float& v, int& len) {
        c = 0;
        v = 0.f;
        len = -1;
        const int e = ft * G + g;
        if (e < n_here) {
            const uint64_t packed = s_seg[wave][fs][e];
            len = (int)(packed >> 58);
            if (li < len) {
                const HopCsr& h = p.hop[SUM ? fs : hop];
                const int64_t at = (int64_t)(packed & kBeginMask) + li;
                c = __builtin_nontemporal_load(h.colidx + at);
                v = __builtin_nontemporal_load(h.vals + at);
            }
        }
        if (++fs == NS) {
            fs = 0;
            ++ft;
        }
    };
#pragma unroll
    for (int k = 0; k < PD; ++k) {
        cq[k] = 0;
        vq[k] = 0.f;
        lq[k] = -1;
        if (k < n_steps) fetch(cq[k], vq[k], lq[k]);
    }
    float part[kTreeParts][VEC];
    int t = 0, s = 0;
    for (int i = 0; i < n_steps; ++i) {
        const int c = cq[0], len = lq[0];
        const float v = vq[0];
#pragma unroll
        for (int k = 0; k + 1 < PD; ++k) {
            cq[k] = cq[k + 1];
            vq[k] = vq[k + 1];
            lq[k] = lq[k + 1];
        }
        lq[PD - 1] = -1;
        if (i + PD < n_steps) fetch(cq[PD - 1], vq[PD - 1], lq[PD - 1]);
        if (s == 0) zero_acc<VEC, kTreeParts>(part);
        int n_max = 0;
#pragma unroll
        for (int gg = 0; gg < G; ++gg) n_max = max(n_max, __builtin_amdgcn_readlane(len, gg * LPR));
        const int hs = SUM ? s : hop;
        const GatherAddr<OFF32> addr{reinterpret_cast<const char*>(p.src + p.src_hop_off[hs] + src_col_begin - VEC), (off_t)lane_off0,
                                     (off_t)(p.ld_src * 4)};
        accumulate_grouped<VEC, LPR, OFF32>(c, v, len, n_max, lane, addr, part);
        if (s == NS - 1) {
            if (len >= 0) {
                float tot[VEC];
                combine_partials<VEC>(part, tot);
                const int64_t row = s_row[wave][t * G + g];
                store_out<VEC, EPI>(p, p.dst + row * p.ld_dst + (SUM ? 0 : p.dst_hop_off[hop]), lcol, ecol, tot);
            }
            s = 0;
            ++t;
        } else {
            ++s;
        }
    }
}

template <int VEC, int LPR, bool SUM, bool OFF32, bool EPI, int MAXB>
__device__ __forceinline__ void medium_list_blocks(const LaunchParams& p, int64_t mblock, int lane, int wave, int64_t lane_off0,
                                                   int64_t src_col_begin, int lcol, int ecol) {
    using off_t = typename std::conditional<OFF32, uint32_t, int64_t>::type;
    constexpr int NP = Tree<LPR>::NP;
    const int g = lane / LPR;
    const int n_sel = p.n_sel;
    int hop = 0;
    int64_t local = mblock;
    if constexpr (!SUM) {
        while (hop + 1 < n_sel && mblock >= p.med_end[hop]) ++hop;
        if (hop > 0) local -= p.med_end[hop - 1];
    }
    const int k = p.med_per_wave;
    const int64_t entry0 = (local * kWavesPerBlock + wave) * k;
    const int64_t left = p.med_count[hop] - entry0;
    if (left <= 0) return;
    const int n_here = left < k ? (int)left : k;
    const int NS = SUM ? n_sel : 1;
    int row = 0;
    int64_t b0 = 0, b1 = 0;
    {
        const int j = lane / NS, s = lane - j * NS;
        if (j < n_here) {
            row = __builtin_nontemporal_load(p.med_list[hop] + entry0 + j);
            const int64_t* rp = p.hop[SUM ? s : hop].rowptr + row;
            b0 = rp[0];
            b1 = rp[1];
        }
    }
    const int b0_lo = (int)(b0 & 0xffffffff), b0_hi = (int)(b0 >> 32), b1_lo = (int)(b1 & 0xffffffff), b1_hi = (int)(b1 >> 32);
    auto bounds = [&](int l, int64_t& sb, int64_t& se) {
        sb = ((int64_t)__builtin_amdgcn_readlane(b0_hi, l) << 32) | (uint32_t)__builtin_amdgcn_readlane(b0_lo, l);
        se = ((int64_t)__builtin_amdgcn_readlane(b1_hi, l) << 32) | (uint32_t)__builtin_amdgcn_readlane(b1_lo, l);
    };
    for (int j = 0; j < n_here; ++j) {
        const int64_t orow = __builtin_amdgcn_readlane(row, j * NS);
        float acc[NP][VEC];
        zero_acc<VEC, NP>(acc);
        for (int s = 0; s < NS; ++s) {
            int64_t sb, se;
            bounds(j * NS + s, sb, se);
            const int hs = SUM ? s : hop;
            const HopCsr& h = p.hop[hs];
            const GatherAddr<OFF32> addr{reinterpret_cast<const char*>(p.src + p.src_hop_off[hs] + src_col_begin - VEC), (off_t)lane_off0,
                                         (off_t)(p.ld_src * 4)};
            accumulate_segment<VEC, LPR, false, OFF32, MAXB>(h.colidx, h.vals, sb, se, 0, 1, addr, lane, true, acc);
        }
        float tot[VEC];
        fold_tree<VEC, LPR, NP>(acc, tot);
        if (g == 0) store_out<VEC, EPI>(p, p.dst + orow * p.ld_dst + (SUM ? 0 : p.dst_hop_off[hop]), lcol, ecol, tot);
    }
}

template <int VEC, int LPR, bool SUM, bool OFF32, bool EPI, int FB>
__device__ __forceinline__ void in_tile_short_rows(const LaunchParams& p, int lane, int rpw, int64_t row0, int rows_here, int rp_lo, int rp_hi,
                                                   int64_t lane_off0_, int64_t src_col_begin, int lcol, int ecol) {
    using off_t = typename std::conditional<OFF32, uint32_t, int64_t>::type;
    constexpr int NP = Tree<LPR>::NP;
    constexpr int kBias = VEC;
    const int li = lane % LPR, g = lane / LPR;
    const int n_sel = p.n_sel;
    const off_t lane_off0 = (off_t)lane_off0_;
    auto seg_bound = [&](int l) -> int64_t {
        return ((int64_t)__builtin_amdgcn_readlane(rp_hi, l) << 32) | (uint32_t)__builtin_amdgcn_readlane(rp_lo, l);
    };
    {
        constexpr int G = kWave / LPR;
        const int short_max = min(LPR, p.long_threshold - 1);
        const int n_blocks = (rows_here + G - 1) / G;
        const GatherAddr<OFF32> addr0{nullptr, lane_off0, (off_t)(p.ld_src * 4)};
        auto row_wave_wide = [&](int r, int s_first, int s_last) {
            float acc[NP][VEC];
            zero_acc<VEC, NP>(acc);
            if constexpr (SUM) {
                for (int s = s_first; s < s_last; ++s) {
                    const int l0 = s * (rpw + 1) + r;
                    if (seg_bound(l0 + 1) - seg_bound(l0) >= p.long_threshold) return;
                }
            }
            for (int s = s_first; s < s_last; ++s) {
                const int l0 = s * (rpw + 1) + r;
                const int64_t sb = seg_bound(l0), se = seg_bound(l0 + 1);
                if (!SUM && se - sb >= p.long_threshold) continue;
                const HopCsr& h = p.hop[s];
                GatherAddr<OFF32> addr = addr0;
                addr.base = reinterpret_cast<const char*>(p.src + p.src_hop_off[s] + src_col_begin - kBias);
                accumulate_segment<VEC, LPR, false, OFF32, FB>(h.colidx, h.vals, sb, se, 0, 1, addr, lane, true, acc);
                if constexpr (!SUM) {
                    float tot[VEC];
                    fold_tree<VEC, LPR, NP>(acc, tot);
                    if (g == 0) store_out<VEC, EPI>(p, p.dst + (row0 + r) * p.ld_dst + p.dst_hop_off[s], lcol, ecol, tot);
                    zero_acc<VEC, NP>(acc);
                }
            }
            if constexpr (SUM) {
                float tot[VEC];
                fold_tree<VEC, LPR, NP>(acc, tot);
                if (g == 0) store_out<VEC, EPI>(p, p.dst + (row0 + r) * p.ld_dst, lcol, ecol, tot);
            }
        };
        auto my_segment = [&](int s, int blk, int64_t& begin, int& len) {
            const int r = blk * G + g;
            const int l0 = s * (rpw + 1) + min(r, rpw - 1);
            const int64_t sb = ((int64_t)lane_gather(rp_hi, l0) << 32) | (uint32_t)lane_gather(rp_lo, l0);
            const int64_t se = ((int64_t)lane_gather(rp_hi, l0 + 1) << 32) | (uint32_t)lane_gather(rp_lo, l0 + 1);
            begin = sb;
            const int64_t n = se - sb;
            len = r < rows_here ? (int)(n > 0x7fffffff ? 0x7fffffff : n) : -1;
        };
        if constexpr (!SUM) {
            const int n_rounds = n_sel * n_blocks;
            int64_t begin_n = 0;
            int len_n = -1, c_n = 0;
            float v_n = 0.f;
            bool short_n = false;
            auto fetch = [&](int i) {
                const int s_ = i / n_blocks, blk_ = i - s_ * n_blocks;
                my_segment(s_, blk_, begin_n, len_n);
                short_n = __builtin_amdgcn_ballot_w64(len_n > short_max) == 0;
                c_n = 0;
                v_n = 0.f;
                if (short_n && li < len_n) {
                    c_n = __builtin_nontemporal_load(p.hop[s_].colidx + begin_n + li);
                    v_n = __builtin_nontemporal_load(p.hop[s_].vals + begin_n + li);
                }
            };
            if (n_rounds > 0) fetch(0);
            for (int i = 0; i < n_rounds; ++i) {
                const int s = i / n_blocks, blk = i - s * n_blocks;
                const int len = len_n, c = c_n;
                const float v = v_n;
                const bool is_short = short_n;
                if (i + 1 < n_rounds) fetch(i + 1);
                if (is_short) {
                    int n_max = 0;
#pragma unroll
                    for (int gg = 0; gg < G; ++gg) n_max = max(n_max, __builtin_amdgcn_readlane(len, gg * LPR));
                    float part[kTreeParts][VEC];
                    zero_acc<VEC, kTreeParts>(part);
                    GatherAddr<OFF32> addr = addr0;
                    addr.base = reinterpret_cast<const char*>(p.src + p.src_hop_off[s] + src_col_begin - kBias);
                    accumulate_grouped<VEC, LPR, OFF32>(c, v, len, n_max, lane, addr, part);
                    float tot[VEC];
                    combine_partials<VEC>(part, tot);
                    if (len >= 0) store_out<VEC, EPI>(p, p.dst + (row0 + blk * G + g) * p.ld_dst + p.dst_hop_off[s], lcol, ecol, tot);
                } else {
                    for (int gg = 0; gg < G && blk * G + gg < rows_here; ++gg) row_wave_wide(blk * G + gg, s, s + 1);
                }
            }
        } else {
            auto block_short = [&](int blk_) {
                bool ok = true;
                for (int s_ = 0; s_ < n_sel; ++s_) {
                    int64_t b_;
                    int l_;
                    my_segment(s_, blk_, b_, l_);
                    ok = ok && __builtin_amdgcn_ballot_w64(l_ > short_max) == 0;
                }
                return ok;
            };
            int64_t begin_n = 0;
            int len_n = -1, c_n = 0;
            float v_n = 0.f;
            auto fetch = [&](int blk_, int s_, bool short_blk) {
                my_segment(s_, blk_, begin_n, len_n);
                c_n = 0;
                v_n = 0.f;
                if (short_blk && li < len_n) {
                    c_n = __builtin_nontemporal_load(p.hop[s_].colidx + begin_n + li);
                    v_n = __builtin_nontemporal_load(p.hop[s_].vals + begin_n + li);
                }
            };
            bool cur_short = n_blocks > 0 && block_short(0);
            if (n_blocks > 0) fetch(0, 0, cur_short);
            for (int blk = 0; blk < n_blocks; ++blk) {
                const bool nxt_short = blk + 1 < n_blocks && block_short(blk + 1);
                if (cur_short) {
                    float part[kTreeParts][VEC];
                    zero_acc<VEC, kTreeParts>(part);
                    bool valid = false;
                    for (int s = 0; s < n_sel; ++s) {
                        const int len = len_n, c = c_n;
                        const float v = v_n;
                        valid = len >= 0;
                        if (s + 1 < n_sel) fetch(blk, s + 1, true);
                        else if (blk + 1 < n_blocks) fetch(blk + 1, 0, nxt_short);
                        int n_max = 0;
#pragma unroll
                        for (int gg = 0; gg < G; ++gg) n_max = max(n_max, __builtin_amdgcn_readlane(len, gg * LPR));
                        GatherAddr<OFF32> addr = addr0;
                        addr.base = reinterpret_cast<const char*>(p.src + p.src_hop_off[s] + src_col_begin - kBias);
                        accumulate_grouped<VEC, LPR, OFF32>(c, v, len, n_max, lane, addr, part);
                    }
                    float tot[VEC];
                    combine_partials<VEC>(part, tot);
                    if (valid) store_out<VEC, EPI>(p, p.dst + (row0 + blk * G + g) * p.ld_dst, lcol, ecol, tot);
                } else {
                    if (blk + 1 < n_blocks) fetch(blk + 1, 0, nxt_short);
                    for (int gg = 0; gg < G && blk * G + gg < rows_here; ++gg) row_wave_wide(blk * G + gg, 0, n_sel);
                }
                cur_short = nxt_short;
            }
        }
        return;
    }
}

template <int VEC, int LPR, bool SUM, bool OFF32, bool PIPE, bool SHORT, bool EPI>
constexpr bool heavy_registers() {
    if (VEC != 4) return false;
    if (SHORT) return (SUM && (!OFF32 || LPR >= 32)) || (!OFF32 && LPR >= 32);
    if (!OFF32) return EPI || LPR >= 32 || PIPE;
    return PIPE && LPR == 32;
}

template <int VEC, int LPR, bool EXACT, bool SUM, bool OFF32, bool PIPE = false, bool SHORT = false, bool EPI = false, int FB = 8, bool LISTS = false>
__global__ __launch_bounds__(kBlock, EXACT ? (LISTS ? (FB == 4 ? H2GCN_SHORT_FB4_MIN_WAVES : heavy_registers<VEC, LPR, SUM, OFF32, PIPE, true, EPI>() ? H2GCN_OFF64_HEAVY_MIN_WAVES : (LPR >= 32 ? H2GCN_WIDE_MIN_WAVES : kMinWavesPerSimd))
                                                : SHORT ? (FB == 4 && !SUM ? H2GCN_SHORT_FB4_MIN_WAVES : H2GCN_SHORT_MIN_WAVES)
                                                : heavy_registers<VEC, LPR, SUM, OFF32, PIPE, false, EPI>() ? H2GCN_OFF64_HEAVY_MIN_WAVES
                                                : (LPR >= 32 ? H2GCN_WIDE_MIN_WAVES : kMinWavesPerSimd)) : 2) void spmm_hops_kernel(const LaunchParams p) {
    static_assert(!LISTS || (EXACT && !SHORT && !PIPE && (LPR == 16 || LPR == 32)), "list-driven launches exist for 64- and 128-column slices");
    static_assert(EXACT || LPR == kWave, "column-tiled path uses the whole wave per row");
    __shared__ float partial[kWavesPerBlock][kMaxTileCols];
    using off_t = typename std::conditional<OFF32, uint32_t, int64_t>::type;
    constexpr int NP = Tree<LPR>::NP;
    constexpr int kMainB = LISTS ? FB : (LPR >= 32 ? H2GCN_WIDE_MAXB : H2GCN_MAIN_MAXB);

    const int lane = threadIdx.x & (kWave - 1);
    const int wave = wave_uniform(threadIdx.x >> 6);
    const int li = lane % LPR;
    const int g = lane / LPR;
    const int n_sel = p.n_sel;

    const int64_t bid = blockIdx.x;
    const int slice = EXACT ? (int)(bid / p.blocks_per_slice) : 0;
    const int64_t b = EXACT ? bid - (int64_t)slice * p.blocks_per_slice : bid;
    const int col_begin = EXACT ? slice * (VEC * LPR) : 0;
    const int col_end = EXACT ? col_begin + VEC * LPR : p.d;
    const int64_t src_col_begin = EXACT ? (int64_t)slice * p.src_slice_stride : 0;
    const int lcol = col_begin + li * VEC;
    const int ecol = EXACT ? ((lcol + VEC <= p.d_src) ? lcol : p.d_src - VEC) : lcol;
    const off_t lane_off0 = (off_t)((ecol - col_begin + VEC) * 4);
    constexpr int kBias = EXACT ? VEC : 0;

    if (b < p.n_long) {
        const int64_t entry = p.long_list[b];
        const int64_t row = SUM ? entry : (entry >> 4);
        const int s_first = SUM ? 0 : (int)(entry & 15);
        const int s_last = SUM ? n_sel : s_first + 1;
        for (int col0 = col_begin; col0 < col_end; col0 += VEC * LPR) {
            const bool lane_active = EXACT || (col0 + li * VEC < p.d);
            float acc[NP][VEC];
            zero_acc<VEC, NP>(acc);
            for (int s = s_first; s < s_last; ++s) {
                const HopCsr& h = p.hop[s];
                const int64_t sb = h.rowptr[row], se = h.rowptr[row + 1];
                const GatherAddr<OFF32> addr{reinterpret_cast<const char*>(p.src + p.src_hop_off[s] + src_col_begin + (col0 - col_begin) - kBias),
                                             EXACT ? lane_off0 : (off_t)(li * VEC * 4), (off_t)(p.ld_src * 4)};
                accumulate_segment<VEC, LPR, !EXACT, OFF32, kMainB>(h.colidx, h.vals, sb, se, wave, kWavesPerBlock, addr, lane,
                                                            lane_active, acc);
            }
            float tot[VEC];
            fold_tree<VEC, LPR, NP>(acc, tot);
            if (g == 0) {
                const int rel = EXACT ? ecol - col_begin : li * VEC;
                if (!EXACT || lcol < p.d_src) {
#pragma unroll
                    for (int i = 0; i < VEC; ++i)
                        if (rel + i >= 0) partial[wave][rel + i] = tot[i];
                }
            }
            __syncthreads();
            const int c = threadIdx.x;
            if (c < VEC * LPR && col0 + c < p.d) {
                float t = partial[0][c];
#pragma unroll
                for (int w = 1; w < kWavesPerBlock; ++w) t += partial[w][c];
                const int64_t off = row * p.ld_dst + (SUM ? 0 : p.dst_hop_off[s_first]) + col0 + c;
                if constexpr (EPI) {
                    if (p.accumulate) t += p.dst[off];
                    if (p.bias) t += p.bias[col0 + c];
                    if (p.relu) t = fmaxf(t, 0.f);
                }
                __builtin_nontemporal_store(t, p.dst + off);
            }
            if (!EXACT) __syncthreads();
        }
        return;
    }

    const int64_t tb = b - p.n_long;
    int64_t tile;
    if constexpr (LISTS) {
        __shared__ uint64_t s_seg[kWavesPerBlock][kShortSumHops][kWave];
        __shared__ int32_t s_row[kWavesPerBlock][kWave];
        const int64_t q = tb >> 3;
        const int i8 = (int)(tb & 7);
        const int64_t n_groups = p.short_groups + p.med_groups;
        const int64_t s_before = (q * p.short_groups) / n_groups;
        if (((q + 1) * p.short_groups) / n_groups > s_before)
            short_list_blocks<VEC, LPR, SUM, OFF32, EPI, H2GCN_SHORT_PREFETCH>(p, s_before * kNumXcd + i8, lane, wave, (int64_t)lane_off0,
                                                                               src_col_begin, lcol, ecol, s_seg, s_row);
        else
            medium_list_blocks<VEC, LPR, SUM, OFF32, EPI, FB>(p, (q - s_before) * kNumXcd + i8, lane, wave, (int64_t)lane_off0,
                                                              src_col_begin, lcol, ecol);
        return;
    } else {
        tile = (tb % kNumXcd) * p.tiles_per_xcd + tb / kNumXcd;
    }
    if (tile >= p.n_tiles) return;
    const int rpw = p.rows_per_wave;
    const int64_t row0 = (tile * kWavesPerBlock + wave) * rpw;
    if (row0 >= p.n_rows) return;
    const int64_t rows_here_l = p.n_rows - row0;
    const int rows_here = rows_here_l < rpw ? (int)rows_here_l : rpw;

    int64_t rp = 0;
    {
        const int hs = lane / (rpw + 1), r = lane % (rpw + 1);
        if (hs < n_sel && r <= rows_here) rp = p.hop[hs].rowptr[row0 + r];
    }
    const int rp_lo = (int)(rp & 0xffffffff), rp_hi = (int)(rp >> 32);
    auto seg_bound = [&](int l) -> int64_t {
        return ((int64_t)__builtin_amdgcn_readlane(rp_hi, l) << 32) | (uint32_t)__builtin_amdgcn_readlane(rp_lo, l);
    };

    if constexpr (SHORT && EXACT && (kWave / LPR == 2 || kWave / LPR == 4)) {
        in_tile_short_rows<VEC, LPR, SUM, OFF32, EPI, FB>(p, lane, rpw, row0, rows_here, rp_lo, rp_hi, (int64_t)lane_off0, src_col_begin, lcol, ecol);
        return;
    }
    if constexpr (PIPE && EXACT) {
        const int n_seg = rows_here * n_sel;
        uint32_t skip = 0;
        for (int q = 0; q < n_seg; ++q) {
            const int r = q / n_sel, s_ = q - r * n_sel;
            const int l0 = s_ * (rpw + 1) + r;
            if (seg_bound(l0 + 1) - seg_bound(l0) >= p.long_threshold) skip |= SUM ? (((1u << n_sel) - 1u) << (r * n_sel)) : (1u << q);
        }
        auto seg = [&](int q, int& s_, int64_t& sb, int64_t& se) {
            const int r = q / n_sel;
            s_ = q - r * n_sel;
            const int l0 = s_ * (rpw + 1) + r;
            sb = seg_bound(l0);
            se = (skip >> q) & 1u ? sb : seg_bound(l0 + 1);
        };
        int s_cur, s_nxt = 0;
        int64_t b_cur, e_cur, b_nxt = 0, e_nxt = 0;
        int c_cur, c_nxt = 0;
        float v_cur, v_nxt = 0.f;
        seg(0, s_nxt, b_nxt, e_nxt);
        load_chunk(p.hop[s_nxt].colidx, p.hop[s_nxt].vals, b_nxt, e_nxt, lane, c_nxt, v_nxt);
        float acc[NP][VEC];
        zero_acc<VEC, NP>(acc);
        for (int q = 0; q < n_seg; ++q) {
            s_cur = s_nxt; b_cur = b_nxt; e_cur = e_nxt; c_cur = c_nxt; v_cur = v_nxt;
            if (q + 1 < n_seg) {
                seg(q + 1, s_nxt, b_nxt, e_nxt);
                load_chunk(p.hop[s_nxt].colidx, p.hop[s_nxt].vals, b_nxt, e_nxt, lane, c_nxt, v_nxt);
            }
            const int r = q / n_sel;
            const int64_t row = row0 + r;
            const HopCsr& h = p.hop[s_cur];
            const GatherAddr<OFF32> addr{reinterpret_cast<const char*>(p.src + p.src_hop_off[s_cur] + src_col_begin - kBias),
                                         lane_off0, (off_t)(p.ld_src * 4)};
            accumulate_segment_prefetched<VEC, LPR, OFF32>(h.colidx, h.vals, b_cur, e_cur, c_cur, v_cur, addr, lane, acc);
            const bool skipped = (skip >> q) & 1u;
            if (!SUM || s_cur == n_sel - 1) {
                if (!skipped) {
                    float tot[VEC];
                    fold_tree<VEC, LPR, NP>(acc, tot);
                    if (g == 0) store_out<VEC, EPI>(p, p.dst + row * p.ld_dst + (SUM ? 0 : p.dst_hop_off[s_cur]), lcol, ecol, tot);
                }
                zero_acc<VEC, NP>(acc);
            }
        }
        return;
    }

#ifdef H2GCN_AB_STORE_BEHIND_FETCH
    if constexpr (EXACT && !SUM && !EPI) {
        float held[VEC];
        int64_t held_off = 0;
        bool held_valid = false;
        for (int r = 0; r < rows_here; ++r) {
            const int64_t row = row0 + r;
            for (int s = 0; s < n_sel; ++s) {
                const int l0 = s * (rpw + 1) + r;
                const int64_t sb = seg_bound(l0), se = seg_bound(l0 + 1);
                if (se - sb >= p.long_threshold) continue;
                const HopCsr& h = p.hop[s];
                int c;
                float v;
                load_chunk(h.colidx, h.vals, sb, se, lane, c, v);
                if (held_valid) {
                    if (g == 0) store_out<VEC, EPI>(p, p.dst + held_off, lcol, ecol, held);
                    held_valid = false;
                }
                float acc[NP][VEC];
                zero_acc<VEC, NP>(acc);
                const GatherAddr<OFF32> addr{reinterpret_cast<const char*>(p.src + p.src_hop_off[s] + src_col_begin - kBias), lane_off0, (off_t)(p.ld_src * 4)};
                accumulate_segment_prefetched<VEC, LPR, OFF32, kMainB>(h.colidx, h.vals, sb, se, c, v, addr, lane, acc);
                fold_tree<VEC, LPR, NP>(acc, held);
                held_off = row * p.ld_dst + p.dst_hop_off[s];
                held_valid = true;
            }
        }
        if (held_valid && g == 0) store_out<VEC, EPI>(p, p.dst + held_off, lcol, ecol, held);
        return;
    }
#endif

    for (int r = 0; r < rows_here; ++r) {
        const int64_t row = row0 + r;
        if constexpr (SUM) {
            bool skip_row = false;
            for (int s = 0; s < n_sel; ++s) {
                const int l0 = s * (rpw + 1) + r;
                const int64_t len = seg_bound(l0 + 1) - seg_bound(l0);
                if (len >= p.long_threshold) skip_row = true;
            }
            if (skip_row) continue;
        }
        for (int col0 = col_begin; col0 < col_end; col0 += VEC * LPR) {
            const bool lane_active = EXACT || (col0 + li * VEC < p.d);
            float acc[NP][VEC];
            zero_acc<VEC, NP>(acc);
#ifdef H2GCN_DEFER_HOP_STORES
            float held[VEC];
            int held_s = -1;
#endif
            for (int s = 0; s < n_sel; ++s) {
                const int l0 = s * (rpw + 1) + r;
                const int64_t sb = seg_bound(l0), se = seg_bound(l0 + 1);
                if (!SUM && se - sb >= p.long_threshold) continue;
                const HopCsr& h = p.hop[s];
                const GatherAddr<OFF32> addr{reinterpret_cast<const char*>(p.src + p.src_hop_off[s] + src_col_begin + (col0 - col_begin) - kBias),
                                             EXACT ? lane_off0 : (off_t)(li * VEC * 4), (off_t)(p.ld_src * 4)};
                accumulate_segment<VEC, LPR, !EXACT, OFF32, kMainB>(h.colidx, h.vals, sb, se, 0, 1, addr, lane, lane_active, acc);
                if constexpr (!SUM) {
                    float tot[VEC];
                    fold_tree<VEC, LPR, NP>(acc, tot);
#ifdef H2GCN_DEFER_HOP_STORES
                    if (EXACT && n_sel == 2 && s == 0) {
#pragma unroll
                        for (int i = 0; i < VEC; ++i) held[i] = tot[i];
                        held_s = 0;
                    } else {
                        if (held_s >= 0 && g == 0 && lane_active)
                            store_out<VEC, EPI>(p, p.dst + row * p.ld_dst + p.dst_hop_off[held_s], lcol, ecol, held);
                        held_s = -1;
                        if (g == 0 && lane_active)
                            store_out<VEC, EPI>(p, p.dst + row * p.ld_dst + p.dst_hop_off[s], EXACT ? lcol : col0 + li * VEC, EXACT ? ecol : col0 + li * VEC, tot);
                    }
#else
                    if (g == 0 && lane_active)
                        store_out<VEC, EPI>(p, p.dst + row * p.ld_dst + p.dst_hop_off[s], EXACT ? lcol : col0 + li * VEC, EXACT ? ecol : col0 + li * VEC, tot);
#endif
                    zero_acc<VEC, NP>(acc);
                }
            }
#ifdef H2GCN_DEFER_HOP_STORES
            if constexpr (!SUM)
                if (held_s >= 0 && g == 0 && lane_active)
                    store_out<VEC, EPI>(p, p.dst + row * p.ld_dst + p.dst_hop_off[held_s], lcol, ecol, held);
#endif
            if constexpr (SUM) {
                float tot[VEC];
                fold_tree<VEC, LPR, NP>(acc, tot);
                if (g == 0 && lane_active)
                    store_out<VEC, EPI>(p, p.dst + row * p.ld_dst, EXACT ? lcol : col0 + li * VEC, EXACT ? ecol : col0 + li * VEC, tot);
            }
        }
    }
}

template <bool VEC4>
__global__ void repack_slice_major_kernel(const float* __restrict__ x, int64_t ld, int64_t ld_hop, int n_hop, int64_t n_rows,
                                          int d, int n_slices, int slice_cols, float* __restrict__ w) {
    using f4 = float __attribute__((ext_vector_type(4)));
    constexpr int E = VEC4 ? 4 : 1;
    const int cu = slice_cols / E;
    const int64_t per_hop = n_rows * cu;
    const int64_t per_slice = per_hop * n_hop;
    const int64_t total = per_slice * n_slices;
    for (int64_t i = (int64_t)blockIdx.x * blockDim.x + threadIdx.x; i < total; i += (int64_t)gridDim.x * blockDim.x) {
        const int q = (int)(i / per_slice);
        const int64_t i1 = i - q * per_slice;
        const int s = (int)(i1 / per_hop);
        const int64_t i2 = i1 - s * per_hop;
        const int64_t r = i2 / cu;
        const int c = (int)(i2 - r * cu);
        const int col = q * slice_cols + c * E;
        const float* src = x + r * ld + s * ld_hop + col;
        if constexpr (VEC4) {
            f4 v = {0.f, 0.f, 0.f, 0.f};
            if (col < d) v = *reinterpret_cast<const f4*>(src);
            __builtin_nontemporal_store(v, reinterpret_cast<f4*>(w) + i);
        } else {
            __builtin_nontemporal_store(col < d ? *src : 0.f, w + i);
        }
    }
}

}
```

### h2gcn_amd/hops.py

```python
from __future__ import annotations

import ctypes as C
from typing import Iterable, Optional, Sequence

import torch

from . import _capi


def _require(cond: bool, msg: str) -> None:
    if not cond:
        raise ValueError(msg)


class HopPlan:

    def __init__(self, rowptr: Sequence[torch.Tensor], colidx: Sequence[torch.Tensor],
                 vals: Sequence[torch.Tensor], n_cols: int, *, build_transpose: bool = False,
                 long_row_threshold: int = 0, rows_per_wave: int = 0, variant: int = 0,
                 slice_cols: int = 0, validate: bool = True, host_transpose: bool = False,
                 keep_permutation: bool = False):
        H = len(rowptr)
        _require(1 <= H <= _capi.MAX_HOPS, f"need 1..{_capi.MAX_HOPS} hop matrices, got {H}")
        _require(len(colidx) == H and len(vals) == H, "rowptr/colidx/vals lists differ in length")
        dev = rowptr[0].device
        _require(dev.type == "cuda", f"HopPlan operands must live on a GPU, got {dev} (no CPU fallback)")
        n_rows = rowptr[0].numel() - 1
        _require(n_rows >= 0, "rowptr must have n_rows+1 entries")
        for k in range(H):
            rp, ci, va = rowptr[k], colidx[k], vals[k]
            _require(rp.dtype == torch.int64 and ci.dtype == torch.int32 and va.dtype == torch.float32,
                     f"hop {k}: dtypes must be int64/int32/float32, got {rp.dtype}/{ci.dtype}/{va.dtype}")
            _require(rp.device == dev and ci.device == dev and va.device == dev, f"hop {k}: operands on different devices")
            _require(rp.dim() == 1 and rp.numel() == n_rows + 1, f"hop {k}: rowptr has {rp.numel()} entries, expected {n_rows + 1}")
            _require(ci.dim() == 1 and va.dim() == 1 and ci.numel() == va.numel(), f"hop {k}: colidx/vals sizes differ")
            _require(rp.is_contiguous() and ci.is_contiguous() and va.is_contiguous(), f"hop {k}: operands must be contiguous")
        self.n_hops = H
        self.n_rows = int(n_rows)
        self.n_cols = int(n_cols)
        self.device = dev
        self.has_transpose = bool(build_transpose)
        self.rowptr = list(rowptr)
        self.colidx = list(colidx)
        self.vals = list(vals)
        self._handle = C.c_void_p()
        self.use_workspace = True
        self.min_chunk_cols = 16

        L = _capi.lib()
        arr_t = C.c_void_p * H
        rp_a = arr_t(*[t.data_ptr() for t in self.rowptr])
        ci_a = arr_t(*[t.data_ptr() for t in self.colidx])
        va_a = arr_t(*[t.data_ptr() for t in self.vals])
        opts = _capi.PlanOpts()
        opts.struct_size = C.sizeof(_capi.PlanOpts)
        opts.flags = ((_capi.PLAN_BUILD_TRANSPOSE if build_transpose else 0) | (0 if validate else _capi.PLAN_SKIP_VALIDATION)
                      | (_capi.PLAN_HOST_TRANSPOSE if host_transpose else 0)
                      | (_capi.PLAN_KEEP_PERMUTATION if keep_permutation and build_transpose else 0))
        opts.long_row_threshold = int(long_row_threshold)
        opts.rows_per_wave = int(rows_per_wave)
        opts.variant = int(variant)
        opts.slice_cols = int(slice_cols)
        with torch.cuda.device(dev):
            stream = torch.cuda.current_stream(dev).cuda_stream
            st = L.h2gcn_plan_create(H, self.n_rows, self.n_cols, rp_a, ci_a, va_a, C.byref(opts),
                                     C.c_void_p(stream), C.byref(self._handle))
        _capi.check(st)

    @classmethod
    def from_scipy(cls, mats: Iterable, device, **kw) -> "HopPlan":
        import numpy as np
        import scipy.sparse as sp

        rowptr, colidx, vals = [], [], []
        n_cols = None
        n_rows = None
        for m in mats:
            m = sp.csr_matrix(m)
            m.sum_duplicates()
            m.sort_indices()
            _require(n_cols in (None, m.shape[1]) and n_rows in (None, m.shape[0]), "hop matrices differ in shape")
            n_rows, n_cols = m.shape
            rowptr.append(torch.from_numpy(m.indptr.astype(np.int64)).to(device))
            colidx.append(torch.from_numpy(m.indices.astype(np.int32)).to(device))
            vals.append(torch.from_numpy(m.data.astype(np.float32)).to(device))
        _require(n_cols is not None, "empty hop list")
        return cls(rowptr, colidx, vals, n_cols, **kw)

    def set_values(self, hop: int, vals: torch.Tensor) -> None:
        _require(vals.dtype == torch.float32 and vals.device == self.device and vals.is_contiguous()
                 and vals.numel() == self.colidx[hop].numel(), "vals must be a contiguous float32 array of the hop's nnz")
        with torch.cuda.device(self.device):
            stream = torch.cuda.current_stream(self.device).cuda_stream
            _capi.check(_capi.lib().h2gcn_plan_set_values(self._handle, int(hop), C.c_void_p(vals.data_ptr()), C.c_void_p(stream)))
        self.vals[hop] = vals
        self.values_version = getattr(self, "values_version", 0) + 1

    @property
    def nnz(self) -> list:
        return [int(t.numel()) for t in self.colidx]

    def info(self, hop: int) -> dict:
        L = _capi.lib()
        n_rows, n_cols, nnz, n_long = C.c_int64(), C.c_int64(), C.c_int64(), C.c_int64()
        has_t = C.c_int32()
        _capi.check(L.h2gcn_plan_info(self._handle, hop, C.byref(n_rows), C.byref(n_cols), C.byref(nnz),
                                      C.byref(n_long), C.byref(has_t)))
        return dict(n_rows=n_rows.value, n_cols=n_cols.value, nnz=nnz.value, n_long_segments=n_long.value,
                    has_transpose=bool(has_t.value))

    def schedule(self, d: int, ld_src: Optional[int] = None, hops=None, adjoint: bool = False) -> dict:
        L = _capi.lib()
        sc, ns, pf, cp = C.c_int32(), C.c_int32(), C.c_int32(), C.c_int32()
        ld = int(ld_src) if ld_src is not None else (self.n_selected(hops) * d if adjoint else d)
        _capi.check(L.h2gcn_plan_schedule(self._handle, self._mask(hops), 1 if adjoint else 0, ld, int(d),
                                          C.byref(sc), C.byref(ns), C.byref(pf), C.byref(cp)))
        return dict(slice_cols=sc.value, n_slices=ns.value,
                    segment_walk={0: "wave per segment", 1: "wave per segment + index prefetch",
                                  2: "lane group per segment (short rows)",
                                  3: "lane group per segment (binned short segments) + wave per segment"}[pf.value],
                    scratch_copy=bool(cp.value) and self.use_workspace)

    def segment_classes(self, d: int, ld_src: Optional[int] = None, hops=None, adjoint: bool = False) -> dict:
        L = _capi.lib()
        if not _capi.has("h2gcn_plan_segment_classes"):
            raise RuntimeError(f"{_capi.library_path()} predates h2gcn_plan_segment_classes (ABI 4)")
        h_sel = self.n_selected(hops)
        seg, nnz, listed = (C.c_int64 * (3 * h_sel))(), (C.c_int64 * (3 * h_sel))(), C.c_int64()
        ld = int(ld_src) if ld_src is not None else (h_sel * d if adjoint else d)
        _capi.check(L.h2gcn_plan_segment_classes(self._handle, self._mask(hops), 1 if adjoint else 0, ld, int(d), seg, nnz, C.byref(listed)))
        sel = list(range(self.n_hops)) if hops is None else sorted({int(h) for h in hops})
        short_walk = ("lane group per segment (binned list)" if listed.value > 0 else
                      "lane group per segment (rounds of consecutive short rows)" if listed.value < 0 else "wave per segment")
        per_hop = [dict(hop=sel[s], segments=dict(short=seg[3 * s], medium=seg[3 * s + 1], long=seg[3 * s + 2]),
                        nonzeros=dict(short=nnz[3 * s], medium=nnz[3 * s + 1], long=nnz[3 * s + 2])) for s in range(h_sel)]
        return dict(per_hop=per_hop, listed=listed.value,
                    walks=dict(short=short_walk, medium="wave per segment", long="workgroup per segment (4 waves, LDS-staged)"))

    def _mask(self, hops) -> int:
        if hops is None:
            return 0
        mask = 0
        for h in hops:
            _require(0 <= int(h) < self.n_hops, f"hop index {h} outside 0..{self.n_hops - 1}")
            mask |= 1 << int(h)
        _require(mask != 0, "empty hop selection")
        return mask

    def n_selected(self, hops) -> int:
        return self.n_hops if hops is None else bin(self._mask(hops)).count("1")

    def spmm(self, x: torch.Tensor, hops=None, out: Optional[torch.Tensor] = None, bias: Optional[torch.Tensor] = None,
             relu: bool = False) -> torch.Tensor:
        _require(x.dim() == 2, f"inputs must be [n_cols, d], got shape {tuple(x.shape)}")
        _require(x.dtype == torch.float32, f"inputs must be float32, got {x.dtype}")
        _require(x.device == self.device, f"inputs on {x.device}, plan on {self.device}")
        _require(x.shape[0] == self.n_cols, f"inputs have {x.shape[0]} rows, hop matrices have {self.n_cols} columns")
        d = int(x.shape[1])
        _require(d >= 1, "inputs need at least one column")
        if x.stride(1) != 1:
            x = x.contiguous()
        h_sel = self.n_selected(hops)
        if out is None:
            out = torch.empty((self.n_rows, h_sel, d), dtype=torch.float32, device=self.device)
        else:
            _require(out.dtype == torch.float32 and out.device == self.device, "out must be float32 on the plan's device")
            _require(tuple(out.shape) == (self.n_rows, h_sel, d), f"out has shape {tuple(out.shape)}, expected {(self.n_rows, h_sel, d)}")
            _require(d == 1 or out.stride(2) == 1, "out's last dimension must be contiguous")
        if self.n_rows == 0:
            return out
        L = _capi.lib()
        mask = self._mask(hops)
        with torch.cuda.device(self.device):
            stream = torch.cuda.current_stream(self.device).cuda_stream
            ws_bytes = int(L.h2gcn_spmm_workspace_bytes(self._handle, mask, 0, C.c_void_p(x.data_ptr()), x.stride(0), 0, d)) if self.use_workspace else 0
            ws = torch.empty(ws_bytes, dtype=torch.uint8, device=self.device) if ws_bytes else None
            opts = None
            if ws is not None or bias is not None or relu:
                if bias is not None:
                    _require(bias.dtype == torch.float32 and bias.device == self.device and bias.numel() == d and bias.is_contiguous(),
                             f"bias must be a contiguous float32 [{d}] tensor on the plan's device")
                opts = _capi.LaunchOpts(struct_size=C.sizeof(_capi.LaunchOpts), flags=_capi.LAUNCH_RELU if relu else 0,
                                        workspace=ws.data_ptr() if ws is not None else None, workspace_bytes=ws_bytes,
                                        bias=bias.data_ptr() if bias is not None else None)
            st = L.h2gcn_spmm_hops_opts_f32(self._handle, mask, C.c_void_p(x.data_ptr()), x.stride(0), d,
                                            C.c_void_p(out.data_ptr()), out.stride(0), out.stride(1) if h_sel > 1 else d,
                                            C.byref(opts) if opts is not None else None, C.c_void_p(stream))
        _capi.check(st)
        return out

    def spmm_t(self, grad: torch.Tensor, hops=None, out: torch.Tensor = None, accumulate: bool = False) -> torch.Tensor:
        _require(self.has_transpose, "plan was built without build_transpose=True; backward is unavailable")
        h_sel = self.n_selected(hops)
        _require(grad.dim() == 3 and grad.shape[0] == self.n_rows and grad.shape[1] == h_sel,
                 f"grad must be [{self.n_rows}, {h_sel}, d], got {tuple(grad.shape)}")
        _require(grad.dtype == torch.float32 and grad.device == self.device, "grad must be float32 on the plan's device")
        d = int(grad.shape[2])
        if grad.stride(2) != 1 or grad.stride(0) < d or (h_sel > 1 and grad.stride(1) < d):
            grad = grad.contiguous()
        if out is None:
            _require(not accumulate, "accumulate=True needs the tensor to accumulate into (out=)")
            dx = torch.empty((self.n_cols, d), dtype=torch.float32, device=self.device)
        else:
            _require(out.shape == (self.n_cols, d) and out.dtype == torch.float32 and out.device == self.device
                     and (out.stride(1) == 1 or d == 1) and (out.stride(0) >= d or self.n_cols <= 1),
                     f"out must be float32 [{self.n_cols}, {d}] on the plan's device with unit column stride")
            dx = out
        if self.n_cols == 0:
            return dx
        L = _capi.lib()
        with torch.cuda.device(self.device):
            stream = torch.cuda.current_stream(self.device).cuda_stream
            mask = self._mask(hops)
            ld_row, ld_hop = (grad.stride(0) if self.n_rows > 0 else h_sel * d), grad.stride(1)
            ws_bytes = int(L.h2gcn_spmm_workspace_bytes(self._handle, mask, 1, C.c_void_p(grad.data_ptr()), ld_row, ld_hop, d)) if self.use_workspace else 0
            opts = None
            if ws_bytes or accumulate:
                ws = torch.empty(ws_bytes, dtype=torch.uint8, device=self.device) if ws_bytes else None
                opts = _capi.LaunchOpts(struct_size=C.sizeof(_capi.LaunchOpts), flags=_capi.LAUNCH_ACCUMULATE if accumulate else 0,
                                        workspace=ws.data_ptr() if ws is not None else None, workspace_bytes=ws_bytes, bias=None)
            st = L.h2gcn_spmm_hops_T_opts_f32(self._handle, mask, C.c_void_p(grad.data_ptr()), ld_row, ld_hop, d,
                                              C.c_void_p(dx.data_ptr()), dx.stride(0) if self.n_cols > 1 else d,
                                              C.byref(opts) if opts is not None else None, C.c_void_p(stream))
        _capi.check(st)
        return dx

    def __del__(self):
        h = getattr(self, "_handle", None)
        if h is not None and h.value:
            try:
                _capi.lib().h2gcn_plan_destroy(h)
            except Exception:
                pass
            self._handle = C.c_void_p()
```

### include/h2gcn_hip.h

```cpp
#ifndef H2GCN_HIP_H_
#define H2GCN_HIP_H_

#include <stddef.h>
#include <stdint.h>

#ifdef __cplusplus
extern "C" {
#endif

#define H2GCN_ABI_VERSION 4
#define H2GCN_MAX_HOPS 8

typedef enum h2gcn_status {
    H2GCN_OK = 0,
    H2GCN_ERR_INVALID_ARGUMENT = -1,
    H2GCN_ERR_HIP = -2,
    H2GCN_ERR_OUT_OF_MEMORY = -3,
    H2GCN_ERR_BAD_INDEX = -4,
    H2GCN_ERR_NO_TRANSPOSE = -5,
    H2GCN_ERR_INTERNAL = -6,
    H2GCN_ERR_EXCHANGE_TIMEOUT = -7
} h2gcn_status;

#define H2GCN_PLAN_BUILD_TRANSPOSE 0x1u
#define H2GCN_PLAN_SKIP_VALIDATION 0x2u
#define H2GCN_PLAN_HOST_TRANSPOSE  0x4u

#define H2GCN_PLAN_KEEP_PERMUTATION 0x8u

typedef struct h2gcn_plan_opts {
    uint32_t struct_size;
    uint32_t flags;
    int32_t long_row_threshold;
    int32_t rows_per_wave;
    int32_t variant;
    int32_t slice_cols;
    int32_t reserved[2];
} h2gcn_plan_opts;

typedef struct h2gcn_plan h2gcn_plan_t;

int h2gcn_abi_version(void);

const char* h2gcn_last_error(void);

int h2gcn_device_count(void);

int h2gcn_plan_create(int n_hops, int64_t n_rows, int64_t n_cols,
                      const int64_t* const* rowptr_dev, const int32_t* const* colidx_dev,
                      const float* const* vals_dev, const h2gcn_plan_opts* opts, void* stream,
                      h2gcn_plan_t** out_plan);

void h2gcn_plan_destroy(h2gcn_plan_t* plan);

int h2gcn_plan_set_values(h2gcn_plan_t* plan, int hop, const float* vals_dev, void* stream);

int h2gcn_plan_info(const h2gcn_plan_t* plan, int hop, int64_t* n_rows, int64_t* n_cols, int64_t* nnz,
                    int64_t* n_long_segments, int32_t* has_transpose);

int h2gcn_plan_schedule(const h2gcn_plan_t* plan, uint32_t hop_mask, int adjoint, int64_t ld_src, int32_t d,
                        int32_t* slice_cols, int32_t* n_slices, int32_t* segment_walk, int32_t* scratch_copy);

int h2gcn_plan_segment_classes(const h2gcn_plan_t* plan, uint32_t hop_mask, int adjoint, int64_t ld_src, int32_t d,
                               int64_t* segments, int64_t* nonzeros, int64_t* listed);

int h2gcn_spmm_hops_f32(const h2gcn_plan_t* plan, uint32_t hop_mask, const float* X_dev, int64_t ldx,
                        int32_t d, float* Y_dev, int64_t ldy_row, int64_t ldy_hop, void* stream);

#define H2GCN_LAUNCH_RELU 0x1u
#define H2GCN_LAUNCH_ACCUMULATE 0x2u
typedef struct h2gcn_launch_opts {
    uint32_t struct_size;
    uint32_t flags;
    void* workspace_dev;
    size_t workspace_bytes;
    const float* bias_dev;
} h2gcn_launch_opts;
size_t h2gcn_spmm_workspace_bytes(const h2gcn_plan_t* plan, uint32_t hop_mask, int adjoint, const float* src_dev,
                                  int64_t ld_src, int64_t ld_src_hop, int32_t d);
int h2gcn_spmm_hops_opts_f32(const h2gcn_plan_t* plan, uint32_t hop_mask, const float* X_dev, int64_t ldx,
                             int32_t d, float* Y_dev, int64_t ldy_row, int64_t ldy_hop,
                             const h2gcn_launch_opts* opts, void* stream);

int h2gcn_spmm_hops_T_f32(const h2gcn_plan_t* plan, uint32_t hop_mask, const float* dY_dev, int64_t ldg_row,
                          int64_t ldg_hop, int32_t d, float* dX_dev, int64_t ldx, void* stream);
int h2gcn_spmm_hops_T_opts_f32(const h2gcn_plan_t* plan, uint32_t hop_mask, const float* dY_dev, int64_t ldg_row,
                               int64_t ldg_hop, int32_t d, float* dX_dev, int64_t ldx,
                               const h2gcn_launch_opts* opts, void* stream);

size_t h2gcn_ring_scratch_bytes(int64_t n);
int h2gcn_ring_count(int64_t n, const int64_t* a_rowptr_dev, const int32_t* a_colidx_dev,
                     const int64_t* f_rowptr_dev, const int32_t* f_colidx_dev,
                     int n_add, const int64_t* const* add_rowptr_dev, const int32_t* const* add_colidx_dev, int add_diag,
                     int n_sub, const int64_t* const* sub_rowptr_dev, const int32_t* const* sub_colidx_dev, int sub_diag,
                     int64_t* out_rowptr_dev, int64_t* nnz_out, void* scratch_dev, size_t scratch_bytes, void* stream);
int h2gcn_ring_fill(int64_t n, const int64_t* a_rowptr_dev, const int32_t* a_colidx_dev,
                    const int64_t* f_rowptr_dev, const int32_t* f_colidx_dev,
                    int n_add, const int64_t* const* add_rowptr_dev, const int32_t* const* add_colidx_dev, int add_diag,
                    int n_sub, const int64_t* const* sub_rowptr_dev, const int32_t* const* sub_colidx_dev, int sub_diag,
                    const int64_t* out_rowptr_dev, int32_t* out_colidx_dev, void* scratch_dev, size_t scratch_bytes,
                    void* stream);
int h2gcn_ring_count_rows(int64_t n, int64_t row_begin, int64_t n_rows, const int64_t* a_rowptr_dev, const int32_t* a_colidx_dev,
                          const int64_t* f_rowptr_dev, const int32_t* f_colidx_dev,
                          int n_add, const int64_t* const* add_rowptr_dev, const int32_t* const* add_colidx_dev, int add_diag,
                          int n_sub, const int64_t* const* sub_rowptr_dev, const int32_t* const* sub_colidx_dev, int sub_diag,
                          int64_t* out_rowptr_dev, int64_t* nnz_out, void* scratch_dev, size_t scratch_bytes, void* stream);
int h2gcn_ring_fill_rows(int64_t n, int64_t row_begin, int64_t n_rows, const int64_t* a_rowptr_dev, const int32_t* a_colidx_dev,
                         const int64_t* f_rowptr_dev, const int32_t* f_colidx_dev,
                         int n_add, const int64_t* const* add_rowptr_dev, const int32_t* const* add_colidx_dev, int add_diag,
                         int n_sub, const int64_t* const* sub_rowptr_dev, const int32_t* const* sub_colidx_dev, int sub_diag,
                         const int64_t* out_rowptr_dev, int32_t* out_colidx_dev, void* scratch_dev, size_t scratch_bytes,
                         void* stream);
int h2gcn_hop_normalize(int64_t n, const int64_t* rowptr_dev, const int32_t* colidx_dev, int mode,
                        const double* s_table_dev, int64_t s_table_len, float* vals_dev, void* stream);
int h2gcn_hop_normalize_rows(int64_t n_rows, const int64_t* rowptr_dev, const int32_t* colidx_dev, int mode,
                             const double* s_table_dev, int64_t s_table_len, const int64_t* col_len_dev,
                             float* vals_dev, void* stream);

int64_t h2gcn_dropout_dense_small_rows(int64_t rows);
size_t h2gcn_dropout_dense_workspace_bytes(int64_t n_rows, int32_t k, int32_t c);
int h2gcn_dropout_dense_f32(const float* X_dev, int64_t ldx, int64_t n_rows, int32_t k, const float* W_dev, int32_t c,
                            const float* bias_dev, float keep_prob, uint64_t seed, const int64_t* step_dev,
                            float* Z_dev, int64_t ldz, void* workspace_dev, size_t workspace_bytes, void* stream);
int h2gcn_dropout_dense_backward_f32(const float* X_dev, int64_t ldx, int64_t n_rows, int32_t k, const float* W_dev, int32_t c,
                                     const float* G_dev, int64_t ldg, float keep_prob, uint64_t seed, const int64_t* step_dev,
                                     float* dX_dev, int64_t lddx, float* dW_dev, void* workspace_dev, size_t workspace_bytes,
                                     void* stream);

#define H2GCN_METRICS_MAX_SETS 4
size_t h2gcn_masked_metrics_workspace_bytes(int64_t n_rows);
int h2gcn_masked_metrics_f32(const float* Z_dev, int64_t ldz, int64_t n_rows, int32_t c, int32_t n_sets, const float* const* Y_dev,
                             const int64_t* ldy, const float* const* w_dev, float* loss_out_dev, float* acc_out_dev,
                             void* workspace_dev, size_t workspace_bytes, void* stream);
int h2gcn_masked_ce_backward_f32(const float* Z_dev, int64_t ldz, int64_t n_rows, int32_t c, const float* Y_dev, int64_t ldy,
                                 const float* w_dev, const float* gscale_dev, float* dZ_dev, int64_t lddz, void* stream);

#define H2GCN_ADAM_MAX_TENSORS 16
int h2gcn_adam_keras_f32(int32_t n_tensors, float* const* params_dev, const float* const* grads_dev, float* const* m_dev,
                         float* const* v_dev, const int64_t* sizes, float lr, float beta1, float beta2, float epsilon,
                         const int64_t* step_dev, int64_t step, void* stream);

int h2gcn_adam_keras_l2_f32(int32_t n_tensors, float* const* params_dev, const float* const* grads_dev, float* const* m_dev,
                            float* const* v_dev, const int64_t* sizes, const float* l2, float lr, float beta_1, float beta_2,
                            float epsilon, const int64_t* step_dev, int64_t step, void* stream);
size_t h2gcn_l2_penalty_workspace_bytes(void);
int h2gcn_l2_penalty_f32(int32_t n_tensors, const float* const* params_dev, const int64_t* sizes, const float* l2,
                         float* out_dev, void* workspace_dev, size_t workspace_bytes, void* stream);

typedef struct h2gcn_xchg h2gcn_xchg_t;

#define H2GCN_XCHG_BLOB_BYTES 192
#define H2GCN_XCHG_COPY_ENGINE 0
#define H2GCN_XCHG_COPY_KERNEL 1

int h2gcn_xchg_create(int world, int rank, int n_channels, size_t slot_bytes, int mode, int timeout_ms,
                      h2gcn_xchg_t** out);
int h2gcn_xchg_export(const h2gcn_xchg_t* x, void* blob_out);
int h2gcn_xchg_connect(h2gcn_xchg_t* x, const void* blobs);
int h2gcn_xchg_allgather_begin(h2gcn_xchg_t* x, int channel, const float* src_dev, int64_t ld_src, int64_t rows,
                               int64_t rows_per_rank, int32_t width, float* full_dev, void* stream);
int h2gcn_xchg_allgather_post(h2gcn_xchg_t* x, int channel, const float* src_dev, int64_t ld_src, int64_t rows,
                              int64_t rows_per_rank, int32_t width, float* full_dev, void* stream);
int h2gcn_xchg_allgather_pull(h2gcn_xchg_t* x, int channel, int64_t rows_per_rank, int32_t width, float* full_dev);
int h2gcn_xchg_allgather_pull_rows(h2gcn_xchg_t* x, int channel, int64_t rows_per_rank, int32_t width, float* full_dev,
                                   const int32_t* const* rows_dev, const int64_t* counts);
int h2gcn_xchg_allgather_end(h2gcn_xchg_t* x, int channel, void* stream);
int h2gcn_xchg_reduce_scatter_begin(h2gcn_xchg_t* x, int channel, const float* src_dev, int64_t rows_per_rank,
                                    int32_t width, float* out_dev, void* stream);
int h2gcn_xchg_reduce_scatter_end(h2gcn_xchg_t* x, int channel, void* stream);
int h2gcn_xchg_reset_dependencies(h2gcn_xchg_t* x);
int h2gcn_xchg_status(const h2gcn_xchg_t* x);
void h2gcn_xchg_destroy(h2gcn_xchg_t* x);

#ifdef __cplusplus
}
#endif
#endif
```

Before: 13.76 billion.

## Stream packed 24-bit column indices and per-row uniform values in forward SpMM

At plan creation, column indices are packed into 16-bit low and 8-bit high arrays, and each row is checked for a single repeated value, which is then stored once per row. Forward, non-sum launches with 4-wide vectors use a compact template path. That path loads the packed indices and broadcasts the per-row value instead of streaming 32-bit indices plus per-edge floats. The aim is to cut index and value bandwidth in the edge stream. The cost is extra plan memory, a host sync whenever values are set, and more kernel instantiations.

```diff
diff --git a/h2gcn_amd/_capi.py b/h2gcn_amd/_capi.py
--- a/h2gcn_amd/_capi.py
+++ b/h2gcn_amd/_capi.py
@@ -25,6 +25,7 @@
 PLAN_SKIP_VALIDATION = 0x2
 PLAN_HOST_TRANSPOSE = 0x4
 PLAN_KEEP_PERMUTATION = 0x8
+PLAN_GENERIC_STREAM = 0x10
 
 EXPORTED_SYMBOLS = (
     "h2gcn_abi_version",
@@ -33,6 +34,7 @@
     "h2gcn_plan_create",
     "h2gcn_plan_destroy",
     "h2gcn_plan_info",
+    "h2gcn_plan_edge_stream",
     "h2gcn_plan_set_values",
     "h2gcn_spmm_hops_f32",
     "h2gcn_spmm_hops_T_f32",
@@ -145,6 +147,8 @@
     L.h2gcn_plan_destroy.argtypes = [C.c_void_p]
     L.h2gcn_plan_set_values.restype = C.c_int
     L.h2gcn_plan_set_values.argtypes = [C.c_void_p, C.c_int, C.c_void_p, C.c_void_p]
+    L.h2gcn_plan_edge_stream.restype = C.c_int
+    L.h2gcn_plan_edge_stream.argtypes = [C.c_void_p, C.c_int, C.POINTER(C.c_int32), C.POINTER(C.c_int32)]
     L.h2gcn_plan_info.restype = C.c_int
     L.h2gcn_plan_info.argtypes = [
         C.c_void_p, C.c_int, C.POINTER(C.c_int64), C.POINTER(C.c_int64), C.POINTER(C.c_int64),
diff --git a/h2gcn_amd/csrc/h2gcn_capi.hip b/h2gcn_amd/csrc/h2gcn_capi.hip
--- a/h2gcn_amd/csrc/h2gcn_capi.hip
+++ b/h2gcn_amd/csrc/h2gcn_capi.hip
@@ -60,6 +60,10 @@
     int64_t n_short = 0, nnz_short = 0;
     int64_t nnz_long = 0;
     const uint32_t* perm = nullptr;
+    const uint16_t* lo16 = nullptr;
+    const uint8_t* hi8 = nullptr;
+    float* row_val = nullptr;
+    bool uniform = false;
 };
 
 struct LongList {
@@ -94,16 +98,34 @@
     mutable std::mutex mu;
     mutable std::map<uint64_t, LongList> long_cache;
     mutable std::map<uint64_t, ClassLists> class_cache;
+    DeviceBuf value_flag;
     int short_max = -1;
     double short_min_frac = 0.05;
 };
 
 namespace h2gcn {
-__global__ void check_colidx_kernel(const int32_t* __restrict__ colidx, int64_t nnz, int64_t n_cols, int* flag) {
+__global__ void check_pack_colidx_kernel(const int32_t* __restrict__ colidx, int64_t nnz, int64_t n_cols, int* flag,
+                                         uint16_t* __restrict__ lo16, uint8_t* __restrict__ hi8) {
     int bad = 0;
     for (int64_t i = (int64_t)blockIdx.x * blockDim.x + threadIdx.x; i < nnz; i += (int64_t)gridDim.x * blockDim.x) {
         const int32_t c = colidx[i];
         bad |= (c < 0) | ((int64_t)c >= n_cols);
+        if (lo16) {
+            lo16[i] = (uint16_t)(c & 0xffff);
+            hi8[i] = (uint8_t)((c >> 16) & 0xff);
+        }
+    }
+    if (flag && bad) atomicOr(flag, 1);
+}
+
+__global__ void derive_row_values_kernel(const int64_t* __restrict__ rowptr, const float* __restrict__ vals, int64_t n_rows,
+                                         float* __restrict__ row_val, int* flag) {
+    int bad = 0;
+    for (int64_t r = (int64_t)blockIdx.x * blockDim.x + threadIdx.x; r < n_rows; r += (int64_t)gridDim.x * blockDim.x) {
+        const int64_t b = rowptr[r], e = rowptr[r + 1];
+        const uint32_t first = b < e ? __float_as_uint(vals[b]) : 0u;
+        for (int64_t j = b + 1; j < e; ++j) bad |= __float_as_uint(vals[j]) != first;
+        row_val[r] = __uint_as_float(first);
     }
     if (bad) atomicOr(flag, 1);
 }
@@ -118,6 +140,7 @@
 namespace {
 
 using h2gcn::HopCsr;
+using h2gcn::CompactCsr;
 using h2gcn::LaunchParams;
 
 int transpose_csr_host(int64_t n_rows, int64_t n_cols, const std::vector<int64_t>& rowptr,
@@ -454,6 +477,8 @@
     } else {
         p.blocks_per_slice = (int64_t)p.n_long + p.tiles_per_xcd * kNumXcd;
     }
+    bool cmp = !SUM;
+    for (int s = 0; s < p.n_sel; ++s) cmp = cmp && p.cmp[s].lo16 && p.cmp[s].row_val;
     const int64_t n_blocks = p.blocks_per_slice * p.n_slices;
     if (n_blocks <= 0) return H2GCN_OK;
     if (n_blocks > 0x7fffffffLL) return fail(H2GCN_ERR_INVALID_ARGUMENT, "grid too large (%lld blocks)", (long long)n_blocks);
@@ -469,25 +494,35 @@
         else                                                                                                                      \
             hipLaunchKernelGGL((spmm_hops_kernel<VEC, LPR, true, SUM, false, false, false, false, 8, true>), grid, block, 0, stream, p);  \
     } while (0)
-#define H2GCN_LAUNCH(VEC, LPR, EXACT)                                                                             \
+#define H2GCN_LAUNCH_CMP(VEC, LPR, EXACT, CMP)                                                                   \
     do {                                                                                                          \
         if (gen && off32)                                                                                         \
-            hipLaunchKernelGGL((spmm_hops_kernel<VEC, LPR, EXACT, SUM, true, false, false, true>), grid, block, 0, stream, p);  \
+            hipLaunchKernelGGL((spmm_hops_kernel<VEC, LPR, EXACT, SUM, true, false, false, true, 8, false, CMP>), grid, block, 0, stream, p);  \
         else if (gen)                                                                                             \
-            hipLaunchKernelGGL((spmm_hops_kernel<VEC, LPR, EXACT, SUM, false, false, false, true>), grid, block, 0, stream, p); \
+            hipLaunchKernelGGL((spmm_hops_kernel<VEC, LPR, EXACT, SUM, false, false, false, true, 8, false, CMP>), grid, block, 0, stream, p); \
         else if (off32 && pipe && EXACT)                                                                               \
-            hipLaunchKernelGGL((spmm_hops_kernel<VEC, LPR, EXACT, SUM, true, true>), grid, block, 0, stream, p);   \
+            hipLaunchKernelGGL((spmm_hops_kernel<VEC, LPR, EXACT, SUM, true, true, false, false, 8, false, CMP>), grid, block, 0, stream, p);   \
         else if (off32)                                                                                           \
-            hipLaunchKernelGGL((spmm_hops_kernel<VEC, LPR, EXACT, SUM, true, false>), grid, block, 0, stream, p);  \
+            hipLaunchKernelGGL((spmm_hops_kernel<VEC, LPR, EXACT, SUM, true, false, false, false, 8, false, CMP>), grid, block, 0, stream, p);  \
         else if (pipe && EXACT)                                                                                   \
-            hipLaunchKernelGGL((spmm_hops_kernel<VEC, LPR, EXACT, SUM, false, true>), grid, block, 0, stream, p);  \
+            hipLaunchKernelGGL((spmm_hops_kernel<VEC, LPR, EXACT, SUM, false, true, false, false, 8, false, CMP>), grid, block, 0, stream, p);  \
         else                                                                                                      \
-            hipLaunchKernelGGL((spmm_hops_kernel<VEC, LPR, EXACT, SUM, false, false>), grid, block, 0, stream, p); \
+            hipLaunchKernelGGL((spmm_hops_kernel<VEC, LPR, EXACT, SUM, false, false, false, false, 8, false, CMP>), grid, block, 0, stream, p); \
+    } while (0)
+#define H2GCN_LAUNCH(VEC, LPR, EXACT) H2GCN_LAUNCH_CMP(VEC, LPR, EXACT, false)
+#define H2GCN_LAUNCH4(LPR)                                                          \
+    do {                                                                            \
+        if constexpr (!SUM) {                                                       \
+            if (cmp) H2GCN_LAUNCH_CMP(4, LPR, true, true);                          \
+            else H2GCN_LAUNCH(4, LPR, true);                                        \
+        } else {                                                                    \
+            H2GCN_LAUNCH(4, LPR, true);                                             \
+        }                                                                           \
     } while (0)
     if (scalar128) {
         H2GCN_LAUNCH(2, 64, true);
     } else if (slice == 256) {
-        H2GCN_LAUNCH(4, 64, true);
+        H2GCN_LAUNCH4(64);
     } else if (slice == 128 && lists) {
         H2GCN_LAUNCH_LISTS(4, 32);
     } else if (slice == 64 && lists) {
@@ -495,13 +530,15 @@
     } else if ((slice == 128 || slice == 64) && shortrow) {
         launch_in_tile_short(SUM, p, slice, off32, short_fb4, grid, stream);
     } else if (slice == 128) {
-        H2GCN_LAUNCH(4, 32, true);
+        H2GCN_LAUNCH4(32);
     } else if (slice == 64) {
-        H2GCN_LAUNCH(4, 16, true);
+        H2GCN_LAUNCH4(16);
     } else {
         H2GCN_LAUNCH(1, 64, false);
     }
+#undef H2GCN_LAUNCH4
 #undef H2GCN_LAUNCH
+#undef H2GCN_LAUNCH_CMP
 #undef H2GCN_LAUNCH_LISTS
     H2GCN_HIP_TRY(hipGetLastError());
     return H2GCN_OK;
@@ -609,6 +646,12 @@
         H2GCN_HIP_TRY(hipMalloc(&flag.p, sizeof(int)));
         H2GCN_HIP_TRY(hipMemsetAsync(flag.p, 0, sizeof(int), stream));
 
+        const bool compact = !(o.flags & H2GCN_PLAN_GENERIC_STREAM) && n_cols <= (1LL << 24);
+        if (compact) {
+            H2GCN_HIP_TRY(hipMalloc(&plan->value_flag.p, n_hops * sizeof(int)));
+            H2GCN_HIP_TRY(hipMemsetAsync(plan->value_flag.p, 0, n_hops * sizeof(int), stream));
+        }
+
         std::vector<std::vector<int64_t>> h_rowptr(n_hops);
         for (int k = 0; k < n_hops; ++k) {
             if (!rowptr_dev[k]) return fail(H2GCN_ERR_INVALID_ARGUMENT, "hop %d: rowptr is NULL", k);
@@ -627,17 +670,43 @@
             if (op.nnz > 0 && (!op.colidx || !op.vals)) return fail(H2GCN_ERR_INVALID_ARGUMENT, "hop %d: colidx/vals is NULL", k);
             collect_long_rows(h_rowptr[k], n_rows, plan->long_threshold, op.long_rows);
             collect_segment_lengths(h_rowptr[k], n_rows, plan->short_max, plan->long_threshold, op);
-            if (!(o.flags & H2GCN_PLAN_SKIP_VALIDATION) && op.nnz > 0) {
+            const bool validate = !(o.flags & H2GCN_PLAN_SKIP_VALIDATION);
+            if (compact && op.nnz > 0) {
+                DeviceBuf lo, hi, rv;
+                if (hipMalloc(&lo.p, op.nnz * sizeof(uint16_t)) == hipSuccess && hipMalloc(&hi.p, op.nnz) == hipSuccess &&
+                    hipMalloc(&rv.p, n_rows * sizeof(float)) == hipSuccess) {
+                    op.lo16 = (const uint16_t*)lo.p;
+                    op.hi8 = (const uint8_t*)hi.p;
+                    op.row_val = (float*)rv.p;
+                    plan->owned.push_back(std::move(lo));
+                    plan->owned.push_back(std::move(hi));
+                    plan->owned.push_back(std::move(rv));
+                } else {
+                    (void)hipGetLastError();
+                }
+            }
+            if ((validate || op.lo16) && op.nnz > 0) {
                 const int64_t want = (op.nnz + 255) / 256;
                 const unsigned blocks = (unsigned)std::min<int64_t>(want, 4096);
-                hipLaunchKernelGGL(h2gcn::check_colidx_kernel, dim3(blocks), dim3(256), 0, stream, op.colidx, op.nnz, n_cols, (int*)flag.p);
+                hipLaunchKernelGGL(h2gcn::check_pack_colidx_kernel, dim3(blocks), dim3(256), 0, stream, op.colidx, op.nnz, n_cols,
+                                   validate ? (int*)flag.p : nullptr, const_cast<uint16_t*>(op.lo16), const_cast<uint8_t*>(op.hi8));
                 H2GCN_HIP_TRY(hipGetLastError());
             }
+            if (op.lo16) {
+                const unsigned blocks = (unsigned)std::min<int64_t>((n_rows + 255) / 256, 4096);
+                hipLaunchKernelGGL(h2gcn::derive_row_values_kernel, dim3(blocks), dim3(256), 0, stream, op.rowptr, op.vals, n_rows,
+                                   op.row_val, (int*)plan->value_flag.p + k);
+                H2GCN_HIP_TRY(hipGetLastError());
+            }
         }
         int h_flag = 0;
+        std::vector<int> h_nonuniform(n_hops, 1);
         H2GCN_HIP_TRY(hipMemcpyAsync(&h_flag, flag.p, sizeof(int), hipMemcpyDeviceToHost, stream));
+        if (compact)
+            H2GCN_HIP_TRY(hipMemcpyAsync(h_nonuniform.data(), plan->value_flag.p, n_hops * sizeof(int), hipMemcpyDeviceToHost, stream));
         H2GCN_HIP_TRY(hipStreamSynchronize(stream));
         if (h_flag) return fail(H2GCN_ERR_BAD_INDEX, "a column index lies outside [0, %lld)", (long long)n_cols);
+        for (int k = 0; k < n_hops; ++k) plan->fwd[k].uniform = plan->fwd[k].lo16 && !h_nonuniform[k];
 
         if (o.flags & H2GCN_PLAN_BUILD_TRANSPOSE) {
             if (n_rows > 0x7fffffffLL) return fail(H2GCN_ERR_INVALID_ARGUMENT, "transpose needs n_rows < 2^31");
@@ -751,7 +820,33 @@
         h2gcn::permute_values(a.perm, vals_dev, a.nnz, const_cast<float*>(a.vals), (hipStream_t)stream_v);
         H2GCN_HIP_TRY(hipGetLastError());
     }
+    if (f.lo16) {
+        hipStream_t stream = (hipStream_t)stream_v;
+        hipStreamCaptureStatus cs = hipStreamCaptureStatusNone;
+        const bool capturing = hipStreamIsCapturing(stream, &cs) == hipSuccess && cs != hipStreamCaptureStatusNone;
+        f.uniform = false;
+        if (!capturing) {
+            int* flag = (int*)plan->value_flag.p + hop;
+            H2GCN_HIP_TRY(hipMemsetAsync(flag, 0, sizeof(int), stream));
+            const unsigned blocks = (unsigned)std::min<int64_t>((plan->n_rows + 255) / 256, 4096);
+            hipLaunchKernelGGL(h2gcn::derive_row_values_kernel, dim3(blocks), dim3(256), 0, stream, f.rowptr, vals_dev, plan->n_rows,
+                               f.row_val, flag);
+            H2GCN_HIP_TRY(hipGetLastError());
+            int h_nonuniform = 1;
+            H2GCN_HIP_TRY(hipMemcpyAsync(&h_nonuniform, flag, sizeof(int), hipMemcpyDeviceToHost, stream));
+            H2GCN_HIP_TRY(hipStreamSynchronize(stream));
+            f.uniform = h_nonuniform == 0;
+        }
+    }
     f.vals = vals_dev;
+    return H2GCN_OK;
+}
+
+int h2gcn_plan_edge_stream(const h2gcn_plan_t* plan, int hop, int32_t* compact_columns, int32_t* row_values) {
+    if (!plan) return fail(H2GCN_ERR_INVALID_ARGUMENT, "plan is NULL");
+    if (hop < 0 || hop >= plan->n_hops) return fail(H2GCN_ERR_INVALID_ARGUMENT, "hop %d outside 0..%d", hop, plan->n_hops - 1);
+    if (compact_columns) *compact_columns = plan->fwd[hop].lo16 ? 1 : 0;
+    if (row_values) *row_values = plan->fwd[hop].uniform ? 1 : 0;
     return H2GCN_OK;
 }
 
@@ -956,6 +1051,7 @@
             if (!(mask & (1u << k))) continue;
             const HopOperand& op = plan->fwd[k];
             p.hop[s] = HopCsr{op.rowptr, op.colidx, op.vals};
+            p.cmp[s] = CompactCsr{op.lo16, op.hi8, op.uniform ? op.row_val : nullptr};
             p.src_hop_off[s] = 0;
             p.dst_hop_off[s] = (int64_t)s * ldy_hop;
             ++s;
diff --git a/h2gcn_amd/csrc/spmm_kernels.hip.h b/h2gcn_amd/csrc/spmm_kernels.hip.h
--- a/h2gcn_amd/csrc/spmm_kernels.hip.h
+++ b/h2gcn_amd/csrc/spmm_kernels.hip.h
@@ -55,6 +55,12 @@
     const int64_t* rowptr;
     const int32_t* colidx;
     const float* vals;
+};
+
+struct CompactCsr {
+    const uint16_t* lo16;
+    const uint8_t* hi8;
+    const float* row_val;
 };
 
 struct LaunchParams {
@@ -94,6 +100,7 @@
     int64_t med_end[H2GCN_MAX_HOPS];
     int64_t med_groups;
     int med_per_wave;
+    CompactCsr cmp[H2GCN_MAX_HOPS];
 };
 
 template <int VEC>
@@ -202,7 +209,7 @@
     }
 };
 
-template <int VEC, int LPR, int U, bool PREDICATED, bool OFF32, int PHASE = 0, int NP>
+template <int VEC, int LPR, int U, bool PREDICATED, bool OFF32, bool CMP, int PHASE = 0, int NP>
 __device__ __forceinline__ void gather_batch(int c, float v, int t, int g, const GatherAddr<OFF32>& addr, bool take,
                                              float (&acc)[NP][VEC]) {
     constexpr int G = kWave / LPR;
@@ -213,11 +220,11 @@
         int cj;
         if constexpr (G == 1) {
             cj = __builtin_amdgcn_readlane(c, t + u);
-            w[u] = __int_as_float(__builtin_amdgcn_readlane(__float_as_int(v), t + u));
+            w[u] = CMP ? v : __int_as_float(__builtin_amdgcn_readlane(__float_as_int(v), t + u));
         } else {
             const int idx = ((t + u) * G + g) & (kWave - 1);
             cj = lane_gather(c, idx);
-            w[u] = lane_gather(v, idx);
+            w[u] = CMP ? v : lane_gather(v, idx);
         }
         const float* p = addr.row(cj);
         if constexpr (PREDICATED) {
@@ -235,72 +242,79 @@
     for (int u = 0; u < U; ++u) fma_vec<VEC>(acc[(PHASE + u) % NP], w[u], x[u]);
 }
 
+template <bool CMP = false>
 __device__ __forceinline__ void load_chunk(const int32_t* __restrict__ colidx, const float* __restrict__ vals,
+                                           const uint16_t* __restrict__ lo16, const uint8_t* __restrict__ hi8,
                                            int64_t base, int64_t seg_end, int lane, int& c, float& v) {
     c = 0;
-    v = 0.f;
+    if constexpr (!CMP) v = 0.f;
     if (base + lane < seg_end) {
-        c = __builtin_nontemporal_load(colidx + base + lane);
-        v = __builtin_nontemporal_load(vals + base + lane);
-    }
-}
-
-template <int VEC, int LPR, bool MASKED, bool OFF32, int MAXB = H2GCN_MAIN_MAXB, int NP>
+        if constexpr (CMP) {
+            c = (int)__builtin_nontemporal_load(lo16 + base + lane) | ((int)__builtin_nontemporal_load(hi8 + base + lane) << 16);
+        } else {
+            c = __builtin_nontemporal_load(colidx + base + lane);
+            v = __builtin_nontemporal_load(vals + base + lane);
+        }
+    }
+}
+
+template <int VEC, int LPR, bool MASKED, bool OFF32, int MAXB = H2GCN_MAIN_MAXB, bool CMP = false, int NP>
 __device__ __forceinline__ void process_chunk(int c, float v, int n, int g, const GatherAddr<OFF32>& addr,
                                               bool lane_active, float (&acc)[NP][VEC]) {
     constexpr int G = kWave / LPR;
     const int full = n / G;
     int t = 0;
     if constexpr (MAXB >= 8)
-        for (; t + 8 <= full; t += 8) gather_batch<VEC, LPR, 8, MASKED, OFF32>(c, v, t, g, addr, lane_active, acc);
+        for (; t + 8 <= full; t += 8) gather_batch<VEC, LPR, 8, MASKED, OFF32, CMP>(c, v, t, g, addr, lane_active, acc);
     if constexpr (MAXB < 8)
-        for (; t + 4 <= full; t += 4) gather_batch<VEC, LPR, 4, MASKED, OFF32>(c, v, t, g, addr, lane_active, acc);
+        for (; t + 4 <= full; t += 4) gather_batch<VEC, LPR, 4, MASKED, OFF32, CMP>(c, v, t, g, addr, lane_active, acc);
     if (t + 4 <= full) {
-        gather_batch<VEC, LPR, 4, MASKED, OFF32>(c, v, t, g, addr, lane_active, acc);
+        gather_batch<VEC, LPR, 4, MASKED, OFF32, CMP>(c, v, t, g, addr, lane_active, acc);
         t += 4;
     }
     const int rem = n - full * G;
     if (t + 2 <= full) {
-        gather_batch<VEC, LPR, 2, MASKED, OFF32>(c, v, t, g, addr, lane_active, acc);
+        gather_batch<VEC, LPR, 2, MASKED, OFF32, CMP>(c, v, t, g, addr, lane_active, acc);
         t += 2;
         if (t + 1 <= full) {
-            gather_batch<VEC, LPR, 1, MASKED, OFF32, 2 % NP>(c, v, t, g, addr, lane_active, acc);
+            gather_batch<VEC, LPR, 1, MASKED, OFF32, CMP, 2 % NP>(c, v, t, g, addr, lane_active, acc);
             if constexpr (G > 1)
-                if (rem > 0) gather_batch<VEC, LPR, 1, true, OFF32, 3 % NP>(c, v, full, g, addr, lane_active && g < rem, acc);
+                if (rem > 0) gather_batch<VEC, LPR, 1, true, OFF32, CMP, 3 % NP>(c, v, full, g, addr, lane_active && g < rem, acc);
         } else {
             if constexpr (G > 1)
-                if (rem > 0) gather_batch<VEC, LPR, 1, true, OFF32, 2 % NP>(c, v, full, g, addr, lane_active && g < rem, acc);
+                if (rem > 0) gather_batch<VEC, LPR, 1, true, OFF32, CMP, 2 % NP>(c, v, full, g, addr, lane_active && g < rem, acc);
         }
     } else if (t + 1 <= full) {
-        gather_batch<VEC, LPR, 1, MASKED, OFF32>(c, v, t, g, addr, lane_active, acc);
+        gather_batch<VEC, LPR, 1, MASKED, OFF32, CMP>(c, v, t, g, addr, lane_active, acc);
         if constexpr (G > 1)
-            if (rem > 0) gather_batch<VEC, LPR, 1, true, OFF32, 1 % NP>(c, v, full, g, addr, lane_active && g < rem, acc);
+            if (rem > 0) gather_batch<VEC, LPR, 1, true, OFF32, CMP, 1 % NP>(c, v, full, g, addr, lane_active && g < rem, acc);
     } else {
         if constexpr (G > 1)
-            if (rem > 0) gather_batch<VEC, LPR, 1, true, OFF32>(c, v, full, g, addr, lane_active && g < rem, acc);
-    }
-}
-
-template <int VEC, int LPR, bool MASKED, bool OFF32, int MAXB = H2GCN_MAIN_MAXB, int NP>
-__device__ __forceinline__ void accumulate_segment(const int32_t* __restrict__ colidx,
-                                                   const float* __restrict__ vals, int64_t seg_begin,
+            if (rem > 0) gather_batch<VEC, LPR, 1, true, OFF32, CMP>(c, v, full, g, addr, lane_active && g < rem, acc);
+    }
+}
+
+template <int VEC, int LPR, bool MASKED, bool OFF32, int MAXB = H2GCN_MAIN_MAXB, bool CMP = false, int NP>
+__device__ __forceinline__ void accumulate_segment(const int32_t* __restrict__ colidx, const float* __restrict__ vals,
+                                                   const uint16_t* __restrict__ lo16, const uint8_t* __restrict__ hi8, int64_t seg_begin,
                                                    int64_t seg_end, int chunk0, int chunk_step,
                                                    const GatherAddr<OFF32>& addr, int lane, bool lane_active,
-                                                   float (&acc)[NP][VEC]) {
+                                                   float (&acc)[NP][VEC], float rv = 0.f) {
     const int g = lane / LPR;
     for (int64_t base = seg_begin + (int64_t)chunk0 * kWave; base < seg_end; base += (int64_t)chunk_step * kWave) {
         const int64_t left = seg_end - base;
         const int n = left < kWave ? (int)left : kWave;
         int c;
-        float v;
-        load_chunk(colidx, vals, base, seg_end, lane, c, v);
-        process_chunk<VEC, LPR, MASKED, OFF32, MAXB>(c, v, n, g, addr, lane_active, acc);
-    }
-}
-
-template <int VEC, int LPR, bool OFF32, int MAXB = H2GCN_MAIN_MAXB, int NP>
-__device__ __forceinline__ void accumulate_segment_prefetched(const int32_t* __restrict__ colidx,
-                                                              const float* __restrict__ vals, int64_t seg_begin,
+        float v = rv;
+        load_chunk<CMP>(colidx, vals, lo16, hi8, base, seg_end, lane, c, v);
+        process_chunk<VEC, LPR, MASKED, OFF32, MAXB, CMP>(c, v, n, g, addr, lane_active, acc);
+    }
+}
+
+template <int VEC, int LPR, bool OFF32, int MAXB = H2GCN_MAIN_MAXB, bool CMP = false, int NP>
+__device__ __forceinline__ void accumulate_segment_prefetched(const int32_t* __restrict__ colidx, const float* __restrict__ vals,
+                                                              const uint16_t* __restrict__ lo16, const uint8_t* __restrict__ hi8,
+                                                              int64_t seg_begin,
                                                               int64_t seg_end, int c, float v,
                                                               const GatherAddr<OFF32>& addr, int lane,
                                                               float (&acc)[NP][VEC]) {
@@ -309,9 +323,9 @@
         const int64_t left = seg_end - base;
         const int n = left < kWave ? (int)left : kWave;
         int c_next = 0;
-        float v_next = 0.f;
-        if (left > kWave) load_chunk(colidx, vals, base + kWave, seg_end, lane, c_next, v_next);
-        process_chunk<VEC, LPR, false, OFF32, MAXB>(c, v, n, g, addr, true, acc);
+        float v_next = CMP ? v : 0.f;
+        if (left > kWave) load_chunk<CMP>(colidx, vals, lo16, hi8, base + kWave, seg_end, lane, c_next, v_next);
+        process_chunk<VEC, LPR, false, OFF32, MAXB, CMP>(c, v, n, g, addr, true, acc);
         c = c_next;
         v = v_next;
     }
@@ -568,7 +582,7 @@
             const HopCsr& h = p.hop[hs];
             const GatherAddr<OFF32> addr{reinterpret_cast<const char*>(p.src + p.src_hop_off[hs] + src_col_begin - VEC), (off_t)lane_off0,
                                          (off_t)(p.ld_src * 4)};
-            accumulate_segment<VEC, LPR, false, OFF32, MAXB>(h.colidx, h.vals, sb, se, 0, 1, addr, lane, true, acc);
+            accumulate_segment<VEC, LPR, false, OFF32, MAXB>(h.colidx, h.vals, nullptr, nullptr, sb, se, 0, 1, addr, lane, true, acc);
         }
         float tot[VEC];
         fold_tree<VEC, LPR, NP>(acc, tot);
@@ -609,7 +623,7 @@
                 const HopCsr& h = p.hop[s];
                 GatherAddr<OFF32> addr = addr0;
                 addr.base = reinterpret_cast<const char*>(p.src + p.src_hop_off[s] + src_col_begin - kBias);
-                accumulate_segment<VEC, LPR, false, OFF32, FB>(h.colidx, h.vals, sb, se, 0, 1, addr, lane, true, acc);
+                accumulate_segment<VEC, LPR, false, OFF32, FB>(h.colidx, h.vals, nullptr, nullptr, sb, se, 0, 1, addr, lane, true, acc);
                 if constexpr (!SUM) {
                     float tot[VEC];
                     fold_tree<VEC, LPR, NP>(acc, tot);
@@ -738,13 +752,15 @@
     return PIPE && LPR == 32;
 }
 
-template <int VEC, int LPR, bool EXACT, bool SUM, bool OFF32, bool PIPE = false, bool SHORT = false, bool EPI = false, int FB = 8, bool LISTS = false>
+template <int VEC, int LPR, bool EXACT, bool SUM, bool OFF32, bool PIPE = false, bool SHORT = false, bool EPI = false, int FB = 8, bool LISTS = false,
+          bool CMP = false>
 __global__ __launch_bounds__(kBlock, EXACT ? (LISTS ? (FB == 4 ? H2GCN_SHORT_FB4_MIN_WAVES : heavy_registers<VEC, LPR, SUM, OFF32, PIPE, true, EPI>() ? H2GCN_OFF64_HEAVY_MIN_WAVES : (LPR >= 32 ? H2GCN_WIDE_MIN_WAVES : kMinWavesPerSimd))
                                                 : SHORT ? (FB == 4 && !SUM ? H2GCN_SHORT_FB4_MIN_WAVES : H2GCN_SHORT_MIN_WAVES)
                                                 : heavy_registers<VEC, LPR, SUM, OFF32, PIPE, false, EPI>() ? H2GCN_OFF64_HEAVY_MIN_WAVES
                                                 : (LPR >= 32 ? H2GCN_WIDE_MIN_WAVES : kMinWavesPerSimd)) : 2) void spmm_hops_kernel(const LaunchParams p) {
     static_assert(!LISTS || (EXACT && !SHORT && !PIPE && (LPR == 16 || LPR == 32)), "list-driven launches exist for 64- and 128-column slices");
     static_assert(EXACT || LPR == kWave, "column-tiled path uses the whole wave per row");
+    static_assert(!CMP || (EXACT && !SUM && !SHORT && !LISTS), "compact stream: forward tile / long / prefetching walks");
     __shared__ float partial[kWavesPerBlock][kMaxTileCols];
     using off_t = typename std::conditional<OFF32, uint32_t, int64_t>::type;
     constexpr int NP = Tree<LPR>::NP;
@@ -781,8 +797,8 @@
                 const int64_t sb = h.rowptr[row], se = h.rowptr[row + 1];
                 const GatherAddr<OFF32> addr{reinterpret_cast<const char*>(p.src + p.src_hop_off[s] + src_col_begin + (col0 - col_begin) - kBias),
                                              EXACT ? lane_off0 : (off_t)(li * VEC * 4), (off_t)(p.ld_src * 4)};
-                accumulate_segment<VEC, LPR, !EXACT, OFF32, kMainB>(h.colidx, h.vals, sb, se, wave, kWavesPerBlock, addr, lane,
-                                                            lane_active, acc);
+                accumulate_segment<VEC, LPR, !EXACT, OFF32, kMainB, CMP>(h.colidx, h.vals, p.cmp[s].lo16, p.cmp[s].hi8, sb, se, wave, kWavesPerBlock, addr, lane,
+                                                                 lane_active, acc, CMP ? p.cmp[s].row_val[row] : 0.f);
             }
             float tot[VEC];
             fold_tree<VEC, LPR, NP>(acc, tot);
@@ -872,22 +888,25 @@
         int64_t b_cur, e_cur, b_nxt = 0, e_nxt = 0;
         int c_cur, c_nxt = 0;
         float v_cur, v_nxt = 0.f;
+        auto seg_val = [&](int q, int s_) { return CMP ? p.cmp[s_].row_val[row0 + q / n_sel] : 0.f; };
         seg(0, s_nxt, b_nxt, e_nxt);
-        load_chunk(p.hop[s_nxt].colidx, p.hop[s_nxt].vals, b_nxt, e_nxt, lane, c_nxt, v_nxt);
+        v_nxt = seg_val(0, s_nxt);
+        load_chunk<CMP>(p.hop[s_nxt].colidx, p.hop[s_nxt].vals, p.cmp[s_nxt].lo16, p.cmp[s_nxt].hi8, b_nxt, e_nxt, lane, c_nxt, v_nxt);
         float acc[NP][VEC];
         zero_acc<VEC, NP>(acc);
         for (int q = 0; q < n_seg; ++q) {
             s_cur = s_nxt; b_cur = b_nxt; e_cur = e_nxt; c_cur = c_nxt; v_cur = v_nxt;
             if (q + 1 < n_seg) {
                 seg(q + 1, s_nxt, b_nxt, e_nxt);
-                load_chunk(p.hop[s_nxt].colidx, p.hop[s_nxt].vals, b_nxt, e_nxt, lane, c_nxt, v_nxt);
+                v_nxt = seg_val(q + 1, s_nxt);
+                load_chunk<CMP>(p.hop[s_nxt].colidx, p.hop[s_nxt].vals, p.cmp[s_nxt].lo16, p.cmp[s_nxt].hi8, b_nxt, e_nxt, lane, c_nxt, v_nxt);
             }
             const int r = q / n_sel;
             const int64_t row = row0 + r;
             const HopCsr& h = p.hop[s_cur];
             const GatherAddr<OFF32> addr{reinterpret_cast<const char*>(p.src + p.src_hop_off[s_cur] + src_col_begin - kBias),
                                          lane_off0, (off_t)(p.ld_src * 4)};
-            accumulate_segment_prefetched<VEC, LPR, OFF32>(h.colidx, h.vals, b_cur, e_cur, c_cur, v_cur, addr, lane, acc);
+            accumulate_segment_prefetched<VEC, LPR, OFF32, H2GCN_MAIN_MAXB, CMP>(h.colidx, h.vals, p.cmp[s_cur].lo16, p.cmp[s_cur].hi8, b_cur, e_cur, c_cur, v_cur, addr, lane, acc);
             const bool skipped = (skip >> q) & 1u;
             if (!SUM || s_cur == n_sel - 1) {
                 if (!skipped) {
@@ -915,7 +934,7 @@
                 const HopCsr& h = p.hop[s];
                 int c;
                 float v;
-                load_chunk(h.colidx, h.vals, sb, se, lane, c, v);
+                load_chunk(h.colidx, h.vals, nullptr, nullptr, sb, se, lane, c, v);
                 if (held_valid) {
                     if (g == 0) store_out<VEC, EPI>(p, p.dst + held_off, lcol, ecol, held);
                     held_valid = false;
@@ -923,7 +942,7 @@
                 float acc[NP][VEC];
                 zero_acc<VEC, NP>(acc);
                 const GatherAddr<OFF32> addr{reinterpret_cast<const char*>(p.src + p.src_hop_off[s] + src_col_begin - kBias), lane_off0, (off_t)(p.ld_src * 4)};
-                accumulate_segment_prefetched<VEC, LPR, OFF32, kMainB>(h.colidx, h.vals, sb, se, c, v, addr, lane, acc);
+                accumulate_segment_prefetched<VEC, LPR, OFF32, kMainB>(h.colidx, h.vals, nullptr, nullptr, sb, se, c, v, addr, lane, acc);
                 fold_tree<VEC, LPR, NP>(acc, held);
                 held_off = row * p.ld_dst + p.dst_hop_off[s];
                 held_valid = true;
@@ -960,7 +979,8 @@
                 const HopCsr& h = p.hop[s];
                 const GatherAddr<OFF32> addr{reinterpret_cast<const char*>(p.src + p.src_hop_off[s] + src_col_begin + (col0 - col_begin) - kBias),
                                              EXACT ? lane_off0 : (off_t)(li * VEC * 4), (off_t)(p.ld_src * 4)};
-                accumulate_segment<VEC, LPR, !EXACT, OFF32, kMainB>(h.colidx, h.vals, sb, se, 0, 1, addr, lane, lane_active, acc);
+                accumulate_segment<VEC, LPR, !EXACT, OFF32, kMainB, CMP>(h.colidx, h.vals, p.cmp[s].lo16, p.cmp[s].hi8, sb, se, 0, 1, addr, lane, lane_active, acc,
+                                                                         CMP ? p.cmp[s].row_val[row] : 0.f);
                 if constexpr (!SUM) {
                     float tot[VEC];
                     fold_tree<VEC, LPR, NP>(acc, tot);
diff --git a/h2gcn_amd/hops.py b/h2gcn_amd/hops.py
--- a/h2gcn_amd/hops.py
+++ b/h2gcn_amd/hops.py
@@ -19,7 +19,7 @@
                  vals: Sequence[torch.Tensor], n_cols: int, *, build_transpose: bool = False,
                  long_row_threshold: int = 0, rows_per_wave: int = 0, variant: int = 0,
                  slice_cols: int = 0, validate: bool = True, host_transpose: bool = False,
-                 keep_permutation: bool = False):
+                 keep_permutation: bool = False, generic_stream: bool = False):
         H = len(rowptr)
         _require(1 <= H <= _capi.MAX_HOPS, f"need 1..{_capi.MAX_HOPS} hop matrices, got {H}")
         _require(len(colidx) == H and len(vals) == H, "rowptr/colidx/vals lists differ in length")
@@ -56,7 +56,8 @@
         opts.struct_size = C.sizeof(_capi.PlanOpts)
         opts.flags = ((_capi.PLAN_BUILD_TRANSPOSE if build_transpose else 0) | (0 if validate else _capi.PLAN_SKIP_VALIDATION)
                       | (_capi.PLAN_HOST_TRANSPOSE if host_transpose else 0)
-                      | (_capi.PLAN_KEEP_PERMUTATION if keep_permutation and build_transpose else 0))
+                      | (_capi.PLAN_KEEP_PERMUTATION if keep_permutation and build_transpose else 0)
+                      | (_capi.PLAN_GENERIC_STREAM if generic_stream else 0))
         opts.long_row_threshold = int(long_row_threshold)
         opts.rows_per_wave = int(rows_per_wave)
         opts.variant = int(variant)
@@ -108,6 +109,11 @@
                                       C.byref(n_long), C.byref(has_t)))
         return dict(n_rows=n_rows.value, n_cols=n_cols.value, nnz=nnz.value, n_long_segments=n_long.value,
                     has_transpose=bool(has_t.value))
+
+    def edge_stream(self, hop: int) -> dict:
+        cc, rv = C.c_int32(), C.c_int32()
+        _capi.check(_capi.lib().h2gcn_plan_edge_stream(self._handle, int(hop), C.byref(cc), C.byref(rv)))
+        return dict(compact_columns=bool(cc.value), row_values=bool(rv.value))
 
     def schedule(self, d: int, ld_src: Optional[int] = None, hops=None, adjoint: bool = False) -> dict:
         L = _capi.lib()
diff --git a/include/h2gcn_hip.h b/include/h2gcn_hip.h
--- a/include/h2gcn_hip.h
+++ b/include/h2gcn_hip.h
@@ -27,6 +27,7 @@
 #define H2GCN_PLAN_HOST_TRANSPOSE  0x4u
 
 #define H2GCN_PLAN_KEEP_PERMUTATION 0x8u
+#define H2GCN_PLAN_GENERIC_STREAM  0x10u
 
 typedef struct h2gcn_plan_opts {
     uint32_t struct_size;
@@ -54,6 +55,8 @@
 void h2gcn_plan_destroy(h2gcn_plan_t* plan);
 
 int h2gcn_plan_set_values(h2gcn_plan_t* plan, int hop, const float* vals_dev, void* stream);
+
+int h2gcn_plan_edge_stream(const h2gcn_plan_t* plan, int hop, int32_t* compact_columns, int32_t* row_values);
 
 int h2gcn_plan_info(const h2gcn_plan_t* plan, int hop, int64_t* n_rows, int64_t* n_cols, int64_t* nnz,
                     int64_t* n_long_segments, int32_t* has_transpose);
```

After: 13.93 billion, median of 6. 1.01x the previous value.
